# nvaccess/NVSpeechPlayer

Hardware: NVIDIA B200
Metric: audio-seconds synthesized/sec (batched streams) (higher is better)
Workload: dtype f32

## Files before the change

### nvspeechplayer_b200/csrc/host.cu

```cuda
#include <chrono>
#include <cstdio>
#include <mutex>
#include <vector>

#include "host.h"

using namespace klatt;

__global__ void init_states_kernel(StreamState *states, uint32_t n) {
	uint32_t i = blockIdx.x * blockDim.x + threadIdx.x;
	if (i >= n) return;
	states[i].fm.lastUserIndex = -1;
	states[i].fm.curIsNull = 1;
	states[i].fm.oldIsNull = 1;
}

namespace klatt {

thread_local std::string g_lastError;

int fail(const std::string &what) {
	g_lastError = what;
	if (envIs("NVSP_VERBOSE")) fprintf(stderr, "[nvspeechplayer_b200] %s\n", what.c_str());
	return -1;
}
void setLastError(const char *what) { fail(what ? what : "error"); }

bool cudaOk(cudaError_t e, const char *what) {
	if (e == cudaSuccess) return true;
	fail(std::string(what) + ": " + cudaGetErrorString(e));
	return false;
}

int pickDevice() {
	static const int chosen = envNum<int>("NVSP_DEVICE", -1);
	int dev = 0;
	if (chosen >= 0) {
		if (cudaSetDevice(chosen) != cudaSuccess) return -1;
		return chosen;
	}
	if (cudaGetDevice(&dev) != cudaSuccess) return -1;
	return dev;
}

int QueueBufs::upload(const void *hFrames, const uint32_t *hMin, const uint32_t *hFade, const int32_t *hUix, const uint8_t *hNull,
                      size_t n, cudaStream_t stream) {
	const size_t m = std::max<size_t>(n, 1);
	if ((hFrames && !frames.reserve(m * kNumParams * sizeof(double))) || (hMin && !minDur.reserve(m * 4)) ||
	    (hFade && !fadeDur.reserve(m * 4)) || (hUix && !userIndex.reserve(m * 4)) || (hNull && !isNull.reserve(m)))
		return -1;
	if (n == 0) return 0;
	if (hFrames) CU(cudaMemcpyAsync(frames.p, hFrames, n * kNumParams * sizeof(double), cudaMemcpyHostToDevice, stream));
	if (hMin) CU(cudaMemcpyAsync(minDur.p, hMin, n * 4, cudaMemcpyHostToDevice, stream));
	if (hFade) CU(cudaMemcpyAsync(fadeDur.p, hFade, n * 4, cudaMemcpyHostToDevice, stream));
	if (hUix) CU(cudaMemcpyAsync(userIndex.p, hUix, n * 4, cudaMemcpyHostToDevice, stream));
	if (hNull) CU(cudaMemcpyAsync(isNull.p, hNull, n, cudaMemcpyHostToDevice, stream));
	return 0;
}

cudaError_t initStates(StreamState *states, uint32_t n, cudaStream_t stream) {
	cudaError_t e = cudaMemsetAsync(states, 0, sizeof(StreamState) * (size_t)n, stream);
	if (e != cudaSuccess) return e;
	init_states_kernel<<<(n + 255) / 256, 256, 0, stream>>>(states, n);
	return cudaGetLastError();
}

bool RoundsCtx::init() {
	if (ok) return true;
	genTicks = std::max<uint32_t>(envNum<uint32_t>("NVSP_GEN_TICKS", 256) & ~63u, 64);
	holdTicks = std::max<uint32_t>(envNum<uint32_t>("NVSP_HOLD_TICKS", 512) & ~63u, 64);
	minStreams = envNum<uint32_t>("NVSP_ROUNDS_MIN_STREAMS", 2048);
	groups = std::min<uint32_t>(std::max<uint32_t>(envNum<uint32_t>("NVSP_GROUPS", 4), 1), kMaxGroups);
	persistent = !envIs("NVSP_SCHED", "rounds");
	blockSched = envIs("NVSP_SCHED", "block");
	blockHoldTicks = std::max<uint32_t>(envNum<uint32_t>("NVSP_BLOCK_HOLD_TICKS", 128) & ~63u, 64);
	blockMinStreams = envNum<uint32_t>("NVSP_BLOCK_MIN_STREAMS", 16384);
	schedGenTicks = std::max<uint32_t>(envNum<uint32_t>("NVSP_SCHED_GEN_TICKS", 384) & ~63u, 64);
	schedHoldTicks = std::max<uint32_t>(envNum<uint32_t>("NVSP_SCHED_HOLD_TICKS", 256) & ~63u, 64);
	schedHoldMax = std::max<uint32_t>(envNum<uint32_t>("NVSP_SCHED_HOLD_MAX", 4096) & ~63u, schedHoldTicks);
	schedFadeTicks = envNum<uint32_t>("NVSP_SCHED_FADE_TICKS", 0) & ~63u;
	schedFadeMax = std::min<uint32_t>(std::max<uint32_t>(envNum<uint32_t>("NVSP_SCHED_FADE_MAX", 512) & ~63u, schedFadeTicks), 4096);
	schedRoleSms = std::min<uint32_t>(envNum<uint32_t>("NVSP_SCHED_HOLD_SMS", 0), 255u) |
	               (std::min<uint32_t>(envNum<uint32_t>("NVSP_SCHED_FADE_SMS", 0), 255u) << 8);
	int dev = 0, sms = 0;
	cudaGetDevice(&dev);
	cudaDeviceGetAttribute(&sms, cudaDevAttrMultiProcessorCount, dev);
	const int perSm = klattF32SchedBlocksPerSm();
	schedBlocks = envNum<uint32_t>("NVSP_SCHED_BLOCKS", (uint32_t)(sms * std::max(perSm, 1)));
	blockBlocks = std::max<uint32_t>(envNum<uint32_t>("NVSP_BLOCK_BLOCKS", (uint32_t)sms), 1);
	if (envIs("NVSP_VERBOSE"))
		fprintf(stderr, "[nvspeechplayer_b200] scheduler: %d SMs x %d blocks, %u blocks, hold %u / general %u ticks\n", sms, perSm,
		        schedBlocks, schedHoldTicks, schedGenTicks);
	if (!cudaOk(cudaEventCreateWithFlags(&evStart, cudaEventDisableTiming), "cudaEventCreate")) return false;
	for (uint32_t g = 0; g < groups; ++g) {
		if (!cudaOk(cudaStreamCreateWithFlags(&lanes[2 * g], cudaStreamNonBlocking), "cudaStreamCreate")) return false;
		if (!cudaOk(cudaStreamCreateWithFlags(&lanes[2 * g + 1], cudaStreamNonBlocking), "cudaStreamCreate")) return false;
		if (!cudaOk(cudaEventCreateWithFlags(&evFork[g], cudaEventDisableTiming), "cudaEventCreate")) return false;
		if (!cudaOk(cudaEventCreateWithFlags(&evJoin[g], cudaEventDisableTiming), "cudaEventCreate")) return false;
	}
	ok = true;
	return true;
}

cudaError_t RoundsCtx::checkFault() {
	if (!hostFault.p) {
		if (hostFault.reserve(sizeof(uint32_t)) != cudaSuccess) return cudaErrorMemoryAllocation;
		*hostFault.as<uint32_t>() = 0;
	}
	return *hostFault.as<uint32_t>() ? cudaErrorLaunchTimeout : cudaSuccess;
}

RoundsCtx::~RoundsCtx() {
	if (evStart) cudaEventDestroy(evStart);
	for (uint32_t g = 0; g < kMaxGroups; ++g) {
		if (evFork[g]) cudaEventDestroy(evFork[g]);
		if (evJoin[g]) cudaEventDestroy(evJoin[g]);
		if (lanes[2 * g]) cudaStreamDestroy(lanes[2 * g]);
		if (lanes[2 * g + 1]) cudaStreamDestroy(lanes[2 * g + 1]);
	}
}

cudaError_t launchRender(int precision, const StreamDesc *descs, uint32_t n, int sampleRate, uint32_t sampleCount,
                         int16_t *out, size_t rowStride, uint32_t *written, StreamResult *results,
                         NoiseConfig noise, cudaStream_t stream, RoundsCtx *rc, bool planned, unsigned long long *launchCounter) {
	if (precision == kPrecisionF64) {
		if (launchCounter) ++*launchCounter;
		return launchKlattF64(descs, n, sampleRate, sampleCount, out, rowStride, written, results, noise, stream);
	}
	if (rc && planned && rc->init() && rc->blockSched && n >= rc->blockMinStreams && klattF32BlockCanTake(n, rc->blockBlocks)) {
		if (!rc->lite.reserve(klattF32BlockLiteBytes(n, rc->blockBlocks)) ||
		    !rc->scratchRow.reserve(sizeof(int16_t) * (size_t)std::max<uint32_t>(std::max(rc->schedHoldTicks, rc->holdTicks), rc->blockHoldTicks)))
			return cudaErrorMemoryAllocation;
		if (!rc->blockProf.p) {
			if (!rc->blockProf.reserve(256)) return cudaErrorMemoryAllocation;
			cudaMemsetAsync(rc->blockProf.p, 0, 256, stream);
		}
		if (cudaError_t e = rc->checkFault()) return e;
		return launchKlattF32Block(descs, n, sampleRate, sampleCount, rc->blockHoldTicks, out, rowStride, written, results, noise,
		                           rc->lite.p, rc->scratchRow.as<int16_t>(), rc->blockBlocks, rc->blockProf.p, rc->hostFault.as<uint32_t>(),
		                           stream, launchCounter);
	}
	if (rc && planned && rc->init() && rc->persistent && n >= rc->minStreams && sampleCount > rc->schedGenTicks) {
		uint32_t cap = 64;
		while (cap < 2 * n) cap <<= 1;
		if (cudaError_t e = rc->checkFault()) return e;
		if (!rc->ring.reserve(sizeof(uint32_t) * 3 * (size_t)cap) || !rc->ctl.reserve(2048) ||
		    !rc->scratchRow.reserve(sizeof(int16_t) * (size_t)std::max(std::max(std::max(rc->schedHoldTicks, rc->schedHoldMax), rc->holdTicks), rc->schedFadeMax)))
			return cudaErrorMemoryAllocation;
		if (klattF32SchedUsesLite() && !rc->lite.reserve(klattF32SchedLiteBytes(n, rc->schedBlocks))) return cudaErrorMemoryAllocation;
		return launchKlattF32Sched(descs, n, sampleRate, sampleCount, rc->schedHoldTicks, rc->schedGenTicks, out, rowStride, written,
		                           results, noise, rc->ring.as<uint32_t>(), cap, rc->ctl.p, rc->scratchRow.as<int16_t>(),
		                           rc->schedBlocks, rc->hostFault.as<uint32_t>(), rc->lite.p, rc->schedHoldMax, rc->schedFadeTicks,
		                           rc->schedFadeMax, rc->schedRoleSms, stream, launchCounter);
	}
	if (rc && planned && rc->init() && n >= rc->minStreams && sampleCount > rc->genTicks) {
		const uint32_t rounds = (sampleCount + rc->genTicks - 1) / rc->genTicks;
		if (!rc->listHold.reserve(sizeof(uint32_t) * (size_t)n) || !rc->listGen.reserve(sizeof(uint32_t) * (size_t)n) ||
		    !rc->counters.reserve(sizeof(uint32_t) * 2 * (size_t)rounds * rc->groups) ||
		    !rc->scratchRow.reserve(sizeof(int16_t) * (size_t)rc->holdTicks))
			return cudaErrorMemoryAllocation;
		return launchKlattF32Rounds(descs, n, sampleRate, sampleCount, rc->holdTicks, rc->genTicks, out, rowStride, written,
		                            results, noise, rc->listHold.as<uint32_t>(), rc->listGen.as<uint32_t>(),
		                            rc->counters.as<uint32_t>(), rc->scratchRow.as<int16_t>(), stream, rc->groups, rc->lanes, rc->evStart, rc->evFork,
		                            rc->evJoin, launchCounter);
	}
	if (launchCounter) ++*launchCounter;
	return launchKlattF32(descs, n, sampleRate, sampleCount, out, rowStride, written, results, noise, stream);
}

bool HostPipe::init() {
	if (ok) return true;
	if (!cudaOk(cudaStreamCreateWithFlags(&compute, cudaStreamNonBlocking), "cudaStreamCreate")) return false;
	if (!cudaOk(cudaStreamCreateWithFlags(&copy, cudaStreamNonBlocking), "cudaStreamCreate")) return false;
	for (int i = 0; i < 2; ++i) {
		if (!cudaOk(cudaEventCreateWithFlags(&kernelDone[i], cudaEventDisableTiming), "cudaEventCreate")) return false;
		if (!cudaOk(cudaEventCreateWithFlags(&copyDone[i], cudaEventDisableTiming), "cudaEventCreate")) return false;
	}
	ok = true;
	return true;
}

HostPipe::~HostPipe() {
	for (int i = 0; i < 2; ++i) {
		if (kernelDone[i]) cudaEventDestroy(kernelDone[i]);
		if (copyDone[i]) cudaEventDestroy(copyDone[i]);
	}
	if (compute) cudaStreamDestroy(compute);
	if (copy) cudaStreamDestroy(copy);
}

static size_t stagingBudgetBytes() {
	const size_t mb = envNum<size_t>("NVSP_STAGE_MB", 2048);
	return std::max<size_t>(mb, 1) << 20;
}

long long renderToHost(HostPipe &pipe, int precision, const StreamDesc *dDescs, uint32_t n, int sampleRate,
                       uint32_t sampleCount, int16_t *hostOut, uint32_t *perStream, StreamResult *lastResults,
                       NoiseConfig noise, unsigned long long *launchCounter, bool planned) {
	if (!pipe.init()) return -1;
	if (n == 0 || sampleCount == 0) return 0;
	size_t budget = stagingBudgetBytes();
	uint64_t maxTicks = std::max<uint64_t>(budget / ((size_t)n * sizeof(int16_t)), 8);
	uint32_t chunk = (uint32_t)std::min<uint64_t>(sampleCount, maxTicks);
	if (chunk < sampleCount) chunk = chunk >= 64 ? (chunk & ~63u) : (chunk & ~7u);
	size_t stride = ((size_t)chunk + 7) & ~(size_t)7;
	for (int i = 0; i < 2; ++i) {
		if (!pipe.stage[i].reserve(stride * n * sizeof(int16_t))) return -1;
		if (!pipe.res[i].reserve((size_t)n * sizeof(StreamResult))) return -1;
	}
	if (!cudaOk(pipe.hostRes.reserve(sizeof(StreamResult) * (size_t)n * 2), "cudaMallocHost")) return -1;
	StreamResult *hostRes = pipe.hostRes.as<StreamResult>();
	std::vector<uint32_t> total(n, 0);
	std::vector<uint32_t> chunkStart, chunkLen;
	{
		uint32_t len = chunk;
		if ((size_t)n * sampleCount * sizeof(int16_t) > ((size_t)256 << 20)) {
			uint64_t first = (((size_t)128 << 20) / ((size_t)n * sizeof(int16_t))) & ~(uint64_t)63;
			len = (uint32_t)std::min<uint64_t>(std::max<uint64_t>(first, 64), chunk);
		}
		for (uint32_t t = 0; t < sampleCount;) {
			uint32_t l = std::min(len, sampleCount - t);
			chunkStart.push_back(t); chunkLen.push_back(l);
			t += l;
			len = std::min<uint32_t>(len * 2, chunk >= 64 ? (chunk & ~63u) : chunk);
		}
	}
	const uint32_t numChunks = (uint32_t)chunkStart.size();
	const bool verbose = envIs("NVSP_VERBOSE");
	auto now = [] { return std::chrono::duration<double, std::milli>(std::chrono::steady_clock::now().time_since_epoch()).count(); };
	const double tStart = now();
	auto harvest = [&](uint32_t c) -> bool {
		int b = c & 1;
		if (!cudaOk(cudaEventSynchronize(pipe.copyDone[b]), "cudaEventSynchronize")) return false;
		const StreamResult *r = hostRes + (size_t)b * n;
		for (uint32_t s = 0; s < n; ++s) total[s] += r[s].written;
		if (lastResults && c + 1 == numChunks) memcpy(lastResults, r, sizeof(StreamResult) * (size_t)n);
		return true;
	};
	std::vector<cudaEvent_t> tev;
	if (verbose) {
		tev.resize(4 * (size_t)numChunks);
		for (auto &e : tev) cudaEventCreate(&e);
	}
	for (uint32_t c = 0; c < numChunks; ++c) {
		int b = c & 1;
		const uint32_t t0 = chunkStart[c], len = chunkLen[c];
		const double tA = now();
		if (c >= 2 && !harvest(c - 2)) return -1;
		const double tB = now();
		if (verbose) cudaEventRecord(tev[4 * c + 0], pipe.compute);
		CU(launchRender(precision, dDescs, n, sampleRate, len, pipe.stage[b].as<int16_t>(), stride, nullptr,
		                pipe.res[b].as<StreamResult>(), noise, pipe.compute, &pipe.rounds, planned, launchCounter));
		if (verbose) cudaEventRecord(tev[4 * c + 1], pipe.compute);
		CU(cudaEventRecord(pipe.kernelDone[b], pipe.compute));
		CU(cudaStreamWaitEvent(pipe.copy, pipe.kernelDone[b], 0));
		if (verbose) cudaEventRecord(tev[4 * c + 2], pipe.copy);
		CU(cudaMemcpy2DAsync(hostOut + t0, (size_t)sampleCount * sizeof(int16_t), pipe.stage[b].p,
		                     stride * sizeof(int16_t), (size_t)len * sizeof(int16_t), n, cudaMemcpyDeviceToHost, pipe.copy));
		CU(cudaMemcpyAsync(hostRes + (size_t)b * n, pipe.res[b].p, sizeof(StreamResult) * (size_t)n,
		                   cudaMemcpyDeviceToHost, pipe.copy));
		if (verbose) cudaEventRecord(tev[4 * c + 3], pipe.copy);
		CU(cudaEventRecord(pipe.copyDone[b], pipe.copy));
		if (verbose) fprintf(stderr, "[renderToHost] chunk %u/%u len %u: t=%.2f ms, waited %.2f ms for chunk-2, enqueue %.2f ms\n", c, numChunks, len,
		                     tA - tStart, tB - tA, now() - tB);
	}
	for (uint32_t c = (numChunks >= 2 ? numChunks - 2 : 0); c < numChunks; ++c)
		if (!harvest(c)) return -1;
	if (verbose) {
		fprintf(stderr, "[renderToHost] done at t=%.2f ms\n", now() - tStart);
		for (uint32_t c = 0; c < numChunks; ++c) {
			float k0, k1, c0, c1;
			cudaEventElapsedTime(&k0, tev[0], tev[4 * c + 0]); cudaEventElapsedTime(&k1, tev[0], tev[4 * c + 1]);
			cudaEventElapsedTime(&c0, tev[0], tev[4 * c + 2]); cudaEventElapsedTime(&c1, tev[0], tev[4 * c + 3]);
			fprintf(stderr, "[renderToHost]   chunk %u: kernel %.2f..%.2f ms, copy %.2f..%.2f ms\n", c, k0, k1, c0, c1);
		}
		for (auto &e : tev) cudaEventDestroy(e);
	}
	long long sum = 0;
	for (uint32_t s = 0; s < n; ++s) {
		sum += total[s];
		if (perStream) perStream[s] = total[s];
	}
	return sum;
}

}
```

### nvspeechplayer_b200/csrc/host.h

```cpp
#pragma once
#include <cuda_runtime.h>
#include <algorithm>
#include <cstdint>
#include <cstdlib>
#include <cstring>
#include <string>

#include "../../include/speechPlayer.h"
#include "klatt_common.h"
#include "launch.h"

namespace klatt {

static_assert(sizeof(speechPlayer_frame_t) == sizeof(double) * kNumParams, "a queued frame is kNumParams doubles");

extern thread_local std::string g_lastError;
int fail(const std::string &what);
void setLastError(const char *what);
bool cudaOk(cudaError_t e, const char *what);
#define CU(call) do { if (!cudaOk((call), #call)) return -1; } while (0)

template <class T = uint64_t> T envNum(const char *name, T dflt) {
	const char *e = getenv(name);
	return (e && *e) ? (T)strtoull(e, nullptr, 0) : dflt;
}
inline bool envIs(const char *name, const char *value = nullptr) {
	const char *e = getenv(name);
	return e && *e && (!value || strcmp(e, value) == 0);
}

int pickDevice();

struct DeviceGuard {
	int prev = -1;
	explicit DeviceGuard(int dev) {
		cudaGetDevice(&prev);
		if (prev != dev) cudaSetDevice(dev);
		else prev = -1;
	}
	~DeviceGuard() {
		if (prev >= 0) cudaSetDevice(prev);
	}
};

struct DevBuf {
	void *p = nullptr;
	size_t cap = 0;
	DevBuf() = default;
	DevBuf(const DevBuf &) = delete;
	DevBuf &operator=(const DevBuf &) = delete;
	DevBuf(DevBuf &&o) noexcept : p(o.p), cap(o.cap) { o.p = nullptr; o.cap = 0; }
	DevBuf &operator=(DevBuf &&o) noexcept { std::swap(p, o.p); std::swap(cap, o.cap); return *this; }
	~DevBuf() {
		if (p) cudaFree(p);
	}
	bool reserve(size_t bytes, const char *what = "cudaMalloc") {
		if (bytes <= cap) return true;
		size_t want = std::max(bytes, cap * 2);
		void *np = nullptr;
		if (!cudaOk(cudaMalloc(&np, want), what)) return false;
		if (p) cudaFree(p);
		p = np; cap = want;
		return true;
	}
	template <class T> T *as() const { return static_cast<T *>(p); }
};

struct PinnedBuf {
	void *p = nullptr;
	size_t cap = 0;
	PinnedBuf() = default;
	PinnedBuf(const PinnedBuf &) = delete;
	PinnedBuf &operator=(const PinnedBuf &) = delete;
	~PinnedBuf() {
		if (p) cudaFreeHost(p);
	}
	cudaError_t reserve(size_t bytes, unsigned flags = cudaHostAllocDefault) {
		if (bytes <= cap) return cudaSuccess;
		if (p) cudaFreeHost(p);
		p = nullptr; cap = 0;
		cudaError_t e = cudaHostAlloc(&p, bytes, flags);
		if (e == cudaSuccess) cap = bytes;
		else p = nullptr;
		return e;
	}
	template <class T> T *as() const { return static_cast<T *>(p); }
};

struct QueueBufs {
	DevBuf frames, minDur, fadeDur, userIndex, isNull;
	int upload(const void *hFrames, const uint32_t *hMin, const uint32_t *hFade, const int32_t *hUix, const uint8_t *hNull, size_t n,
	           cudaStream_t stream);
};

inline unsigned long long timelineTicks(const unsigned int *minDur, const unsigned int *fadeDur, size_t n) {
	unsigned long long t = 0;
	for (size_t i = 0; i < n; ++i) {
		unsigned long long m = minDur[i], f = fadeDur[i] > 1 ? fadeDur[i] : 1;
		t += std::max(m + 1, f + 2);
	}
	return t;
}

cudaError_t initStates(StreamState *states, uint32_t n, cudaStream_t stream);

struct RoundsCtx {
	static constexpr uint32_t kMaxGroups = 8;
	DevBuf listHold, listGen, counters, scratchRow;
	DevBuf ring, ctl;
	bool persistent = true;
	DevBuf lite, blockProf;
	bool blockSched = false;
	uint32_t blockHoldTicks = 128, blockMinStreams = 16384, blockBlocks = 0;
	PinnedBuf hostFault;
	uint32_t schedHoldTicks = 256, schedGenTicks = 384, schedHoldMax = 4096, schedFadeTicks = 0, schedFadeMax = 512, schedRoleSms = 0, schedBlocks = 0;
	cudaStream_t lanes[2 * kMaxGroups] = {};
	cudaEvent_t evStart = nullptr, evFork[kMaxGroups] = {}, evJoin[kMaxGroups] = {};
	uint32_t holdTicks = 512, genTicks = 256, minStreams = 2048, groups = 4;
	bool ok = false;
	bool init();
	cudaError_t checkFault();
	~RoundsCtx();
};

cudaError_t launchRender(int precision, const StreamDesc *descs, uint32_t n, int sampleRate, uint32_t sampleCount,
                         int16_t *out, size_t rowStride, uint32_t *written, StreamResult *results,
                         NoiseConfig noise, cudaStream_t stream, RoundsCtx *rc = nullptr, bool planned = false,
                         unsigned long long *launchCounter = nullptr);

struct HostPipe {
	cudaStream_t compute = nullptr, copy = nullptr;
	cudaEvent_t kernelDone[2] = {nullptr, nullptr}, copyDone[2] = {nullptr, nullptr};
	DevBuf stage[2], res[2];
	RoundsCtx rounds;
	PinnedBuf hostRes;
	bool ok = false;
	bool init();
	~HostPipe();
};

long long renderToHost(HostPipe &pipe, int precision, const StreamDesc *dDescs, uint32_t n, int sampleRate,
                       uint32_t sampleCount, int16_t *hostOut, uint32_t *perStream, StreamResult *lastResults,
                       NoiseConfig noise, unsigned long long *launchCounter, bool planned = false);

}
```

### nvspeechplayer_b200/csrc/klatt_f32_core.cuh

```cuda
#pragma once
#include <math.h>
#include <stdint.h>
#include <string.h>
#include <type_traits>
#include "klatt_common.h"
#include "philox.cuh"

#if defined(__GNUC__) || defined(__CUDACC__)
#define KLATT_UNLIKELY(x) __builtin_expect(!!(x), 0)
#else
#define KLATT_UNLIKELY(x) (x)
#endif

namespace klatt {

enum Direct : int {
	dVibratoPitchOffset = 0, dVoiceTurbulenceAmplitude, dGlottalOpenQuotient, dVoiceAmplitude,
	dAspirationAmplitude, dCaNP, dPa1, dPa2, dPa3, dPa4, dPa5, dPa6, dFricationAmplitude, dParallelBypass,
	dPreFormantGain, dOutputGain
};
static_assert(dOutputGain + 1 == kNumDirect, "direct slots");

KLATT_HD constexpr int directParam(int i) {
	return i == dVibratoPitchOffset ? kVibratoPitchOffset
	     : i == dVoiceTurbulenceAmplitude ? kVoiceTurbulenceAmplitude : i == dGlottalOpenQuotient ? kGlottalOpenQuotient
	     : i == dVoiceAmplitude ? kVoiceAmplitude : i == dAspirationAmplitude ? kAspirationAmplitude
	     : i == dCaNP ? kCaNP : i == dFricationAmplitude ? kFricationAmplitude
	     : (i >= dPa1 && i <= dPa6) ? (kPa1 + (i - dPa1))
	     : i == dParallelBypass ? kParallelBypass : i == dPreFormantGain ? kPreFormantGain : kOutputGain;
}

KLATT_HD void oneMinusExpD(double x, double th, double &re, double &im) {
	double em1 = expm1(x);
	double r = 1.0 + em1;
	double sh, ch;
	sincos(0.5 * th, &sh, &ch);
	re = -em1 + 2.0 * r * sh * sh;
	im = -r * (2.0 * sh * ch);
}
KLATT_HD void oneMinusExp(double x, double th, float &re, float &im) {
	double dre, dim;
	oneMinusExpD(x, th, dre, dim);
	re = (float)dre;
	im = (float)dim;
}
KLATT_HD void poleTerms(double f, double bw, double srInv, float &zre, float &zim) {
	const double PI = 3.14159265358979323846;
	oneMinusExp(-PI * bw * srInv , 2.0 * PI * f * srInv , zre, zim);
}

KLATT_HD int64_t vibratoIncrement(double speed, double srInv) {
	double t = speed * srInv;
	if (t != t) t = 0.0;
	if (!(t > -0.49 && t < 0.49)) t = fmod(t, 1.0);
	if (t >= 0.5) t -= 1.0;
	if (t < -0.5) t += 1.0;
	return (int64_t)(t * 18446744073709551616.0);
}

constexpr double kSinTurnsGain = 1.0 + 3.861e-8;
KLATT_HD double vibratoDepth(double vibratoPitchOffset) { return vibratoPitchOffset * (0.06 / kSinTurnsGain); }

KLATT_HD void planFade(const double *o, const double *n, uint32_t F, int sampleRate, FadePlanF32 &p) {
	const double srInv = 1.0 / (double)sampleRate;
	const double invF = 1.0 / (double)F;
	{
		double v0 = o[kVibratoSpeed], v1 = n[kVibratoSpeed];
		if (v1 != v1) v1 = v0;
		p.vibInc0 = vibratoIncrement(v0, srInv);
		p.vibIncFinal = vibratoIncrement(v0 + ((v1 - v0) * 1.0), srInv);
		p.vibIncStep = (p.vibIncFinal - p.vibInc0) / (int64_t)F;
		double d0 = o[kVibratoPitchOffset], d1 = n[kVibratoPitchOffset];
		if (d1 != d1) d1 = d0;
		p.depth0 = vibratoDepth(d0);
		p.depthStep = vibratoDepth((d1 - d0) * invF);
		p.depthFinal = vibratoDepth(d0 + ((d1 - d0) * 1.0));
	}
	for (int i = 0; i < kNumDirect; ++i) {
		double a = o[directParam(i)], b = n[directParam(i)];
		if (b != b) b = a;
		p.dir0[i] = (float)a;
		p.dirStep[i] = (float)((b - a) * invF);
		p.dirFinal[i] = (float)(a + ((b - a) * 1.0));
	}
	for (int r = 0; r < kNumResonators; ++r) {
		double f0 = o[resFreqParam(r)], f1 = n[resFreqParam(r)];
		double b0 = o[resBwParam(r)], b1 = n[resBwParam(r)];
		if (f1 != f1) f1 = f0;
		if (b1 != b1) b1 = b0;
		poleTerms(f0, b0, srInv, p.z0re[r], p.z0im[r]);
		poleTerms(f0 + ((f1 - f0) * 1.0), b0 + ((b1 - b0) * 1.0), srInv, p.zFre[r], p.zFim[r]);
		const double PI = 3.14159265358979323846;
		double xs = -PI * (b1 - b0) * invF * srInv;
		double dth = 2.0 * PI * (f1 - f0) * invF * srInv;
		double wr, wi;
		oneMinusExpD(xs, dth, wr, wi);
		p.wre[r] = (float)wr; p.wim[r] = (float)wi;
		static_assert(kCoarseTicks == 64, "six squarings");
#pragma unroll
		for (int k = 0; k < 6; ++k) {
			const double ar = 2.0 - wr, ai = -wi;
			const double nr = wr * ar - wi * ai, ni = wr * ai + wi * ar;
			wr = nr; wi = ni;
		}
		p.Wre[r] = (float)wr; p.Wim[r] = (float)wi;
		if (r == kResN0) {
			p.n0InvFade = !(f0 == 0 && f1 == 0);
			p.n0InvFinal = (f0 + ((f1 - f0) * 1.0)) != 0;
		}
	}
}

KLATT_HD void plannedFrames(const double *prevReal, bool prevIsNull, const double *cur, bool curIsNull, double *o, double *n) {
	for (int i = 0; i < kNumParams; ++i) o[i] = prevReal ? prevReal[i] : 0.0;
	if (prevIsNull) o[kPreFormantGain] = 0;
	if (curIsNull) {
		for (int i = 0; i < kNumParams; ++i) n[i] = o[i];
		n[kPreFormantGain] = 0;
	} else {
		for (int i = 0; i < kNumParams; ++i) n[i] = cur[i];
		if (prevIsNull) {
			for (int i = 0; i < kNumParams; ++i) o[i] = n[i];
			o[kPreFormantGain] = 0;
		}
	}
}

enum Role : int { kRoleBoth = 0, kRoleCascade = 1, kRoleParallel = 2, kRoleCascadeOsc = 3, kRoleParallelOnly = 4 };
constexpr int kGroupTicks = 8;
#ifndef KLATT_HOLD_UNROLL
#define KLATT_HOLD_UNROLL 1
#endif
constexpr int kHoldUnroll = KLATT_HOLD_UNROLL;

template <int ROLE> struct RoleTraits {
	static constexpr bool hasC = ROLE == kRoleBoth || ROLE == kRoleCascade || ROLE == kRoleCascadeOsc;
	static constexpr bool hasP = ROLE == kRoleBoth || ROLE == kRoleParallel || ROLE == kRoleParallelOnly;
	static constexpr bool hasO = ROLE == kRoleBoth || ROLE == kRoleParallel || ROLE == kRoleCascadeOsc;
	static constexpr int R0 = hasC ? 0 : kResParallel;
	static constexpr int R1 = hasP ? kNumResonators : kResParallel;
};
KLATT_HD constexpr bool directOfCascade(int i) {
	return i == dVoiceTurbulenceAmplitude || i == dGlottalOpenQuotient || i == dVoiceAmplitude ||
	       i == dAspirationAmplitude || i == dCaNP || i == dPreFormantGain || i == dOutputGain;
}
KLATT_HD constexpr bool directOfParallel(int i) {
	return i == dFricationAmplitude || (i >= dPa1 && i <= dPa6) || i == dParallelBypass || i == dPreFormantGain;
}
template <int ROLE> KLATT_HD constexpr bool roleUsesDirect(int i) {
	return (RoleTraits<ROLE>::hasC && directOfCascade(i)) || (RoleTraits<ROLE>::hasP && directOfParallel(i));
}

struct XchgSelf {
	uint32_t wA_;
	float par_, voice_;
	KLATT_HD void put(uint32_t, uint32_t wA, float par, float voice) { wA_ = wA; par_ = par; voice_ = voice; }
	KLATT_HD void get(uint32_t, uint32_t &wA, float &par, float &voice) const { wA = wA_; par = par_; voice = voice_; }
	KLATT_HD void sync() {}
};

struct F2 { float lo, hi; };
KLATT_HD F2 f2(float lo, float hi) { F2 r; r.lo = lo; r.hi = hi; return r; }
KLATT_HD F2 f2s(float x) { F2 r; r.lo = x; r.hi = x; return r; }
KLATT_HD F2 fma2(F2 a, F2 b, F2 c) {
	F2 r;
#ifdef __CUDA_ARCH__
	asm("{ .reg .b64 pa, pb, pc, pd; mov.b64 pa, {%2, %3}; mov.b64 pb, {%4, %5}; mov.b64 pc, {%6, %7}; "
	    "fma.rn.f32x2 pd, pa, pb, pc; mov.b64 {%0, %1}, pd; }"
	    : "=f"(r.lo), "=f"(r.hi) : "f"(a.lo), "f"(a.hi), "f"(b.lo), "f"(b.hi), "f"(c.lo), "f"(c.hi));
#else
	r.lo = fmaf(a.lo, b.lo, c.lo); r.hi = fmaf(a.hi, b.hi, c.hi);
#endif
	return r;
}
KLATT_HD F2 mul2(F2 a, F2 b) {
	F2 r;
#ifdef __CUDA_ARCH__
	asm("{ .reg .b64 pa, pb, pd; mov.b64 pa, {%2, %3}; mov.b64 pb, {%4, %5}; mul.rn.f32x2 pd, pa, pb; mov.b64 {%0, %1}, pd; }"
	    : "=f"(r.lo), "=f"(r.hi) : "f"(a.lo), "f"(a.hi), "f"(b.lo), "f"(b.hi));
#else
	r.lo = a.lo * b.lo; r.hi = a.hi * b.hi;
#endif
	return r;
}
KLATT_HD F2 add2(F2 a, F2 b) {
	F2 r;
#ifdef __CUDA_ARCH__
	asm("{ .reg .b64 pa, pb, pd; mov.b64 pa, {%2, %3}; mov.b64 pb, {%4, %5}; add.rn.f32x2 pd, pa, pb; mov.b64 {%0, %1}, pd; }"
	    : "=f"(r.lo), "=f"(r.hi) : "f"(a.lo), "f"(a.hi), "f"(b.lo), "f"(b.hi));
#else
	r.lo = a.lo + b.lo; r.hi = a.hi + b.hi;
#endif
	return r;
}
KLATT_HD F2 sub2(F2 a, F2 b) {
	F2 r;
#ifdef __CUDA_ARCH__
	asm("{ .reg .b64 pa, pb, pd; mov.b64 pa, {%2, %3}; mov.b64 pb, {%4, %5}; sub.rn.f32x2 pd, pa, pb; mov.b64 {%0, %1}, pd; }"
	    : "=f"(r.lo), "=f"(r.hi) : "f"(a.lo), "f"(a.hi), "f"(b.lo), "f"(b.hi));
#else
	r.lo = a.lo - b.lo; r.hi = a.hi - b.hi;
#endif
	return r;
}
KLATT_HD float &half(F2 *arr, int r) { return (r & 1) ? arr[r >> 1].hi : arr[r >> 1].lo; }
KLATT_HD const float &half(const F2 *arr, int r) { return (r & 1) ? arr[r >> 1].hi : arr[r >> 1].lo; }

constexpr int kNumPairs = kNumResonators / 2;
constexpr int kNumDirectPairs = kNumDirect / 2;
static_assert(kResCascade % 2 == 0 && kResParallel % 2 == 0, "role boundaries fall between pairs");
template <int ROLE> struct PairTraits {
	static constexpr int P0 = RoleTraits<ROLE>::R0 / 2, P1 = RoleTraits<ROLE>::R1 / 2;
};
template <int ROLE> KLATT_HD constexpr bool roleUsesDirectPair(int k) {
	return roleUsesDirect<ROLE>(2 * k) || roleUsesDirect<ROLE>(2 * k + 1);
}

struct DspState {
	F2 ny[kNumPairs];
	F2 d[kNumPairs];
	float aspLast, fricLast;
	uint64_t vibratoPos;
	int64_t vibInc;
	double pitchPos;
	double pitch, pitchInc;
	double depth;
};

struct CoefF32 {
	F2 a[kNumPairs], nrho[kNumPairs];
	float invA0;
	float vta, goq, va, aa, caNP, bypass;
	F2 pa[3];
	float halfGain, fricGain, og4000;
	bool n0Inv;
};

KLATT_HD float fastRcp(float x) {
#ifdef __CUDA_ARCH__
	float r;
	asm("rcp.approx.ftz.f32 %0, %1;" : "=f"(r) : "f"(x));
	return r;
#else
	return 1.0f / x;
#endif
}

constexpr float kDrawScale = 1.0f / 8388608.0f;

template <int ROLE>
KLATT_HD void buildCoef(CoefF32 &C, const F2 *u, const F2 *v, const F2 *dir, bool n0Inv) {
	using T = RoleTraits<ROLE>;
	using P = PairTraits<ROLE>;
#pragma unroll
	for (int k = P::P0; k < P::P1; ++k) {
		F2 a = fma2(u[k], u[k], mul2(v[k], v[k]));
		C.a[k] = a;
		C.nrho[k] = fma2(f2s(2.0f), u[k], a);
	}
	C.halfGain = half(dir, dPreFormantGain) * 0.5f;
	if (T::hasC) {
		C.invA0 = fastRcp(C.a[0].lo);
		C.vta = half(dir, dVoiceTurbulenceAmplitude); C.goq = half(dir, dGlottalOpenQuotient);
		C.va = half(dir, dVoiceAmplitude); C.aa = half(dir, dAspirationAmplitude); C.caNP = half(dir, dCaNP);
		C.og4000 = half(dir, dOutputGain) * 4000.0f;
		C.n0Inv = n0Inv;
	}
	if (T::hasP) {
		static_assert(dPa1 % 2 == 0, "the parallel amplitudes are whole pairs of the direct params");
#pragma unroll
		for (int k = 0; k < 3; ++k) C.pa[k] = dir[dPa1 / 2 + k];
		C.bypass = half(dir, dParallelBypass);
		C.fricGain = ((0.3f * kDrawScale) * half(dir, dFricationAmplitude)) * C.halfGain;
	}
}

template <int ROLE>
KLATT_HD void stepPoles(F2 *u, F2 *v, const F2 *wr, const F2 *wi) {
	using P = PairTraits<ROLE>;
#pragma unroll
	for (int k = P::P0; k < P::P1; ++k) {
		F2 zi = mul2(v[k], f2s(-1.0f));
		F2 tr = fma2(u[k], wr[k], wr[k]);
		tr = fma2(zi, wi[k], tr);
		F2 ti = fma2(u[k], wi[k], wi[k]);
		ti = fma2(v[k], wr[k], ti);
		u[k] = sub2(u[k], tr);
		v[k] = sub2(v[k], ti);
	}
}

KLATT_HD float sectionOut(float &ny, float &d, float a, float w, float x) {
	float dn = fmaf(a, x, w);
	d = dn;
	ny = ny - dn;
	return -ny;
}
KLATT_HD F2 sectionMemory(const DspState &S, const CoefF32 &C, int k) {
	F2 w = fma2(C.nrho[k], S.d[k], S.d[k]);
	return fma2(C.a[k], S.ny[k], w);
}

KLATT_HD float sinTurns(float t) {
	if (t > 0.25f) t = 0.5f - t;
	if (t < -0.25f) t = -0.5f - t;
	const float u = t * t;
	float q = fmaf(u, -14.3368558883667f, 41.999961853027344f);
	q = fmaf(u, q, -76.70366668701172f);
	q = fmaf(u, q, 81.60520935058594f);
	q = fmaf(u, q, -41.34170150756836f);
	return fmaf(t * u, q, t * 6.2831854820251465f);
}

KLATT_HD float bitsToFloat(uint32_t u) {
#ifdef __CUDA_ARCH__
	return __uint_as_float(u);
#else
	float f;
	memcpy(&f, &u, 4);
	return f;
#endif
}

KLATT_HD int64_t cyclesToFixed(double x) {
#ifdef __CUDA_ARCH__
	return __double2ll_rn(x * 18446744073709551616.0);
#else
	double y = x * 18446744073709551616.0;
	if (y != y) return (int64_t)0x8000000000000000ull;
	if (y >= 9223372036854775807.0) return 0x7fffffffffffffffll;
	if (y <= -9223372036854775808.0) return (int64_t)0x8000000000000000ull;
	return (int64_t)nearbyint(y);
#endif
}

KLATT_HD double fracRef(double x) {
#ifdef __CUDA_ARCH__
	if (fabs(x) < 2.0) {
		double t = x >= 1.0 ? 1.0 : 0.0;
		t = x <= -1.0 ? -1.0 : t;
		return x - t;
	}
	return x - (double)__double2int_rz(x);
#else
	double t = (x != x) ? 0.0 : (x >= 2147483647.0 ? 2147483647.0 : (x <= -2147483648.0 ? -2147483648.0 : (double)(int32_t)x));
	return x - t;
#endif
}

KLATT_HD double glideExact(double p, double inc, uint64_t n) {
	if (n == 0) return p;
	if (!(inc == inc) || !(p == p) || inc == 0.0) return p + inc;
	while (n > 0) {
		const double p1 = p + inc;
		if (--n == 0) return p1;
		const double p2 = p1 + inc;
		if (--n == 0) return p2;
		const double p3 = p2 + inc;
		--n;
		p = p3;
		if (n == 0) return p3;
		const double step = p3 - p2;
		if (step == 0.0) return p3;
		const double a1 = p1 < 0 ? -p1 : p1, a2 = p2 < 0 ? -p2 : p2, a3 = p3 < 0 ? -p3 : p3;
		if (!(a3 >= 1e-290 && a3 <= 1e290) || !(a2 >= 1e-290) || !(a1 >= 1e-290)) continue;
		int e1, e2, e3;
		(void)frexp(a1, &e1);
		(void)frexp(a2, &e2);
		const double f3 = frexp(a3, &e3);
		if (e1 != e3 || e2 != e3 || (p1 < 0) != (p3 < 0) || (p2 < 0) != (p3 < 0)) continue;
		const int64_t P = (int64_t)ldexp(f3, 53);
		const double sMag = ldexp(step, 53 - e3);
		const int64_t S = (p3 < 0) ? -(int64_t)sMag : (int64_t)sMag;
		if (S == 0) continue;
		const int64_t lo = (int64_t)1 << 52, hi = (int64_t)1 << 53;
		int64_t room = S > 0 ? (hi - P) / S : (P - lo) / (-S);
		room -= 1;
		if (room <= 0) continue;
		const uint64_t k = (uint64_t)room < n ? (uint64_t)room : n;
		const double mag = ldexp((double)(P + (int64_t)k * S), e3 - 53);
		p = (p3 < 0) ? -mag : mag;
		n -= k;
	}
	return p;
}

KLATT_HD float parallelSide(DspState &S, const CoefF32 &C, uint32_t wF) {
	float uF = bitsToFloat(0x4B000000u | (wF >> 9)) - 8388608.0f;
	S.fricLast = fmaf(0.75f, S.fricLast, uF);
	float pin = S.fricLast * C.fricGain;
	const F2 pin2 = f2s(pin);
	F2 nacc = f2s(0.0f);
#pragma unroll
	for (int k = 0; k < 3; ++k) {
		const int p = kResParallel / 2 + k;
		F2 dn = fma2(C.a[p], pin2, sectionMemory(S, C, p));
		S.d[p] = dn;
		S.ny[p] = sub2(S.ny[p], dn);
		nacc = fma2(add2(S.ny[p], pin2), C.pa[k], nacc);
	}
	float par = -(nacc.lo + nacc.hi);
	return fmaf(pin - par, C.bypass, par);
}

KLATT_HD double divideBySampleRate(double x, double srD, double srInv) {
	double q = x * srInv;
	double r = fma(-q, srD, x);
	return fma(r, srInv, q);
}

struct OscChain {
	float t, u, q;
	double m, quot, pos;
	KLATT_HD void seg1(DspState &S) {
		S.vibratoPos += (uint64_t)S.vibInc;
		t = (float)(int32_t)(uint32_t)(S.vibratoPos >> 32) * 2.3283064365386963e-10f;
		if (t > 0.25f) t = 0.5f - t;
		if (t < -0.25f) t = -0.5f - t;
		u = t * t;
	}
	KLATT_HD void seg2() {
		q = fmaf(u, -14.3368558883667f, 41.999961853027344f);
		q = fmaf(u, q, -76.70366668701172f);
		q = fmaf(u, q, 81.60520935058594f);
		q = fmaf(u, q, -41.34170150756836f);
		q = fmaf(t * u, q, t * 6.2831854820251465f);
	}
	KLATT_HD void seg3(DspState &S) {
		S.pitch += S.pitchInc;
		m = S.pitch * fma((double)q, S.depth, 1.0);
	}
	KLATT_HD void seg4(double srD, double srInv) { quot = divideBySampleRate(m, srD, srInv); }
	KLATT_HD void seg5(DspState &S) {
		pos = fracRef(quot + S.pitchPos);
		S.pitchPos = pos;
	}
	KLATT_HD float seg6() const { return (float)pos; }
};

KLATT_HD float oscillatorSide(DspState &S, const CoefF32 &C, double srD, double srInv) {
	OscChain o;
	o.seg1(S); o.seg2(); o.seg3(S); o.seg4(srD, srInv); o.seg5(S);
	return o.seg6();
}

KLATT_HD float stageSource(DspState &S, const CoefF32 &C, uint32_t wA, float voice) {
	float uA = bitsToFloat(0x4B000000u | (wA >> 9)) - 8388608.0f;
	S.aspLast = fmaf(0.75f, S.aspLast, uA);
	float asp = S.aspLast * (0.2f * kDrawScale);
	float turb = asp * C.vta;
	if (voice < C.goq) turb *= 0.01f;
	float v = (fmaf(voice, 2.0f, -1.0f) + turb) * C.va;
	float src = fmaf(asp, C.aa, v);
	return src * C.halfGain;
}
KLATT_HD float stageNasal(DspState &S, const CoefF32 &C, float ci) {
	float dx = ci - S.ny[0].lo;
	float dx1 = fmaf(C.nrho[0].lo, S.d[0].lo, S.d[0].lo);
	float n0 = C.n0Inv ? fmaf(dx - dx1, C.invA0, S.ny[0].lo)
	                   : fmaf(C.a[0].lo, dx, dx1 + S.ny[0].lo);
	S.d[0].lo = dx;
	S.ny[0].lo = ci;
	float wNP = fmaf(C.nrho[0].hi, S.d[0].hi, S.d[0].hi);
	wNP = fmaf(C.a[0].hi, S.ny[0].hi, wNP);
	float np = sectionOut(S.ny[0].hi, S.d[0].hi, C.a[0].hi, wNP, n0);
	return fmaf(np - ci, C.caNP, ci);
}
KLATT_HD float stageSection(DspState &S, const CoefF32 &C, int q, float w, float x) {
	const int r = kResCascade + q;
	return sectionOut(half(S.ny, r), half(S.d, r), half(C.a, r), w, x);
}
KLATT_HD int stageOut(const CoefF32 &C, float x, float par) {
	float s = (x + par) * C.og4000;
	s = fminf(s, 32000.0f);
	s = fmaxf(s, -32000.0f);
	return (int)s;
}

KLATT_HD int cascadeSide(DspState &S, const CoefF32 &C, uint32_t wA, float par, float voice) {
	float ci = stageSource(S, C, wA, voice);
	F2 w[3];
#pragma unroll
	for (int p = 0; p < 3; ++p) w[p] = sectionMemory(S, C, 1 + p);
	float x = stageNasal(S, C, ci);
#pragma unroll
	for (int q = 0; q < 6; ++q) x = stageSection(S, C, q, half(w, q), x);
	return stageOut(C, x, par);
}

struct NoiseSource {
	Philox4 blk;
	uint64_t blkIndex;
	KLATT_HD void init() { blk.w[0] = blk.w[1] = blk.w[2] = blk.w[3] = 0; blkIndex = ~0ull; }
	KLATT_HD void draw(const NoiseConfig &noise, const StreamDesc &desc, uint64_t streamId, uint64_t gen, uint32_t &wA, uint32_t &wF) {
		if (noise.mode == kNoisePhilox) {
			uint64_t b = gen >> 1;
			if (b != blkIndex) { blk = noiseBlock(noise.seed, streamId, b); blkIndex = b; }
			bool odd = (gen & 1ull) != 0;
			wA = odd ? blk.w[2] : blk.w[0];
			wF = odd ? blk.w[3] : blk.w[1];
		} else {
			uint64_t d0 = 2 * gen - desc.replayBase;
			wA = (d0 < desc.replayLen) ? ((uint32_t)desc.replay[d0] << 1) : 0u;
			wF = (d0 + 1 < desc.replayLen) ? ((uint32_t)desc.replay[d0 + 1] << 1) : 0u;
		}
	}
};

template <int ROLE, class GS>
KLATT_HD void loadDspState(DspState &S, const GS &gs) {
	using T = RoleTraits<ROLE>;
#pragma unroll
	for (int r = T::R0; r < T::R1; ++r) { half(S.ny, r) = (r == kResN0) ? gs.y[r] : -gs.y[r]; half(S.d, r) = gs.d[r]; }
	if (T::hasC) S.aspLast = gs.aspLast;
	if (T::hasP) S.fricLast = gs.fricLast;
	if (T::hasO) {
		S.vibratoPos = gs.vibratoPos; S.vibInc = gs.vibInc;
		S.pitchPos = gs.pitchPos; S.pitch = gs.pitch; S.pitchInc = gs.pitchInc; S.depth = gs.depth;
	}
}
template <int ROLE, class GS>
KLATT_HD void storeDspState(GS &gs, const DspState &S) {
	using T = RoleTraits<ROLE>;
#pragma unroll
	for (int r = T::R0; r < T::R1; ++r) { gs.y[r] = (r == kResN0) ? half(S.ny, r) : -half(S.ny, r); gs.d[r] = half(S.d, r); }
	if (T::hasC) gs.aspLast = S.aspLast;
	if (T::hasP) gs.fricLast = S.fricLast;
	if (T::hasO) {
		gs.vibratoPos = S.vibratoPos; gs.vibInc = S.vibInc;
		gs.pitchPos = S.pitchPos; gs.pitch = S.pitch; gs.pitchInc = S.pitchInc; gs.depth = S.depth;
	}
}

template <class FM, class GS>
KLATT_HD bool canHoldF32T(const FM &fm, const GS &gs, uint32_t ticks) {
	return !fm.hasNew && !fm.curIsNull && !fm.purgePending && gs.holdArmed && (uint64_t)fm.counter + ticks <= (uint64_t)fm.oldM;
}
KLATT_HD bool canHoldF32(const StreamState &st, uint32_t ticks) { return canHoldF32T(st.fm, st.gen.f32, ticks); }
template <class FM, class GS>
KLATT_HD bool canFadeF32T(const FM &fm, const GS &gs, uint32_t ticks) {
	return fm.hasNew && !fm.purgePending && fm.counter >= 1 && (uint64_t)fm.counter + ticks < (uint64_t)fm.newF &&
	       (gs.samplesGenerated & (uint64_t)(kCoarseTicks - 1)) == 0;
}

template <int ROLE, class Out, class Xchg, class FM, class GS>
KLATT_HD void renderHoldF32T(FM &fm, GS &gs, const StreamDesc &desc, int sampleRate, uint32_t ticks, Out &out, const NoiseConfig &noise,
                             Xchg &xc) {
	using T = RoleTraits<ROLE>;
	const double srD = (double)sampleRate, srInv = 1.0 / (double)sampleRate;
	DspState S;
	loadDspState<ROLE>(S, gs);
	CoefF32 C;
	{
		F2 u[kNumPairs], v[kNumPairs], dir[kNumDirectPairs];
#pragma unroll
		for (int r = T::R0; r < T::R1; ++r) { half(u, r) = -gs.zre[r]; half(v, r) = -gs.zim[r]; }
#pragma unroll
		for (int i = 0; i < kNumDirect; ++i)
			if (roleUsesDirectPair<ROLE>(i / 2)) half(dir, i) = roleUsesDirect<ROLE>(i) ? gs.dir[i] : 0.0f;
		buildCoef<ROLE>(C, u, v, dir, gs.n0Inv != 0);
	}
	uint64_t gen = gs.samplesGenerated;
	const uint64_t streamId = desc.streamId;
	NoiseSource ns;
	ns.init();
	const bool evenPhilox = noise.mode == kNoisePhilox && (gen & 1ull) == 0;
	for (uint32_t t = 0; t < ticks; t += kGroupTicks) {
		if (T::hasC && !T::hasP) xc.sync();
		if (!T::hasP || evenPhilox) {
#pragma unroll(kHoldUnroll)
			for (int k = 0; k < kGroupTicks; k += 2) {
				Philox4 blk;
				if (T::hasP) blk = noiseBlock(noise.seed, streamId, (gen + k) >> 1);
#pragma unroll
				for (int h = 0; h < 2; ++h) {
					uint32_t wA = 0;
					float par = 0.0f, voice = 0.0f;
					if (T::hasP) {
						wA = blk.w[2 * h];
						par = parallelSide(S, C, blk.w[2 * h + 1]);
						if (T::hasO && !T::hasC) voice = oscillatorSide(S, C, srD, srInv);
						if (!T::hasC) xc.put(t + k + h, wA, par, voice);
					}
					if (T::hasC) {
						if (!T::hasP) xc.get(t + k + h, wA, par, voice);
						if (T::hasO) voice = oscillatorSide(S, C, srD, srInv);
						out.push(cascadeSide(S, C, wA, par, voice));
					}
				}
			}
		} else {
			for (int k = 0; k < kGroupTicks; ++k) {
				uint32_t wA, wF;
				ns.draw(noise, desc, streamId, gen + k, wA, wF);
				float par = parallelSide(S, C, wF), voice = 0.0f;
				if (T::hasO) voice = oscillatorSide(S, C, srD, srInv);
				if (!T::hasC) xc.put(t + k, wA, par, voice);
				if (T::hasC) out.push(cascadeSide(S, C, wA, par, voice));
			}
		}
		gen += kGroupTicks;
		if (T::hasP && !T::hasC) xc.sync();
	}
	storeDspState<ROLE>(gs, S);
	if (T::hasC) {
		gs.samplesGenerated = gen;
		fm.counter += ticks;
		gs.callPos += ticks;
	}
}
template <int ROLE, class Out, class Xchg>
KLATT_HD void renderHoldF32(const StreamDesc &desc, int sampleRate, uint32_t ticks, Out &out, const NoiseConfig &noise, Xchg &xc) {
	renderHoldF32T<ROLE>(desc.state->fm, desc.state->gen.f32, desc, sampleRate, ticks, out, noise, xc);
}

template <int ROLE, class Out, class Xchg, class FM, class GS>
KLATT_HD uint32_t renderGeneralF32T(FM &fm, GS &gs, const StreamDesc &desc, int sampleRate, uint32_t myTicks, uint32_t loopTicks, Out &out,
                                    const NoiseConfig &noise, Xchg &xc, int32_t *lastUserIndexOut, uint32_t *qHeadOut) {
	using T = RoleTraits<ROLE>;
	constexpr bool kInline = ROLE == kRoleBoth && std::is_same<FM, FrameMgrState>::value;
	const double srD = (double)sampleRate, srInv = 1.0 / (double)sampleRate;
	const bool planned = desc.plans != nullptr;

	uint32_t counter = fm.counter, qHead = fm.qHead;
	uint32_t oldM = fm.oldM, newM = fm.newM, newF = fm.newF;
	int32_t lastUserIndex = fm.lastUserIndex;
	bool hasNew = fm.hasNew, curIsNull = fm.curIsNull, oldIsNull = fm.oldIsNull, newIsNull = fm.newIsNull;
	uint32_t nextEvent = gs.nextEvent;
	bool holdArmed = gs.holdArmed != 0;
	bool n0Inv = gs.n0Inv != 0;

	DspState S;
	loadDspState<ROLE>(S, gs);
	using P = PairTraits<ROLE>;
	F2 u[kNumPairs], v[kNumPairs], wr[kNumPairs], wi[kNumPairs];
	F2 dir0[kNumDirectPairs], dstep[kNumDirectPairs];
	float kf = 0.0f, kfStep = 0.0f;
	int64_t vibIncStep = 0;
	double depthStep = 0.0;
#pragma unroll
	for (int r = T::R0; r < T::R1; ++r) { half(u, r) = -gs.zre[r]; half(v, r) = -gs.zim[r]; half(wr, r) = 0.0f; half(wi, r) = 0.0f; }
#pragma unroll
	for (int i = 0; i < kNumDirect; ++i)
		if (roleUsesDirectPair<ROLE>(i / 2)) { half(dir0, i) = roleUsesDirect<ROLE>(i) ? gs.dir[i] : 0.0f; half(dstep, i) = 0.0f; }
	uint64_t gen = gs.samplesGenerated;
	const uint64_t streamId = desc.streamId;

	if constexpr (kInline) {
		if (fm.purgePending) {
			fm.purgePending = 0;
			counter = oldM;
			if (hasNew) {
				oldIsNull = newIsNull;
				for (int i = 0; i < kNumParams; ++i) fm.oldFrame[i] = fm.curFrame[i];
				hasNew = false;
			}
			S.pitchInc = 0.0;
			holdArmed = false;
			nextEvent = oldM + 1;
		}
	}
	const FadePlanF32 *plan = nullptr;
	if (hasNew) {
		if constexpr (kInline) plan = planned ? desc.plans + (qHead - 1 - desc.qBase) : &gs.plan;
		else plan = desc.plans + (qHead - 1 - desc.qBase);
		if (counter >= 1 && counter < newF) {
#pragma unroll
			for (int r = T::R0; r < T::R1; ++r) { half(wr, r) = plan->wre[r]; half(wi, r) = plan->wim[r]; }
#pragma unroll
			for (int i = 0; i < kNumDirect; ++i)
				if (roleUsesDirect<ROLE>(i)) { half(dir0, i) = plan->dir0[i]; half(dstep, i) = plan->dirStep[i]; }
			kf = (float)counter;
			kfStep = 1.0f;
			vibIncStep = plan->vibIncStep;
			depthStep = plan->depthStep;
		}
	}
	uint32_t coarseAt = hasNew ? gs.coarseAt : 0x80000000u;

	NoiseSource ns;
	ns.init();

	uint32_t produced = 0;
	bool active = myTicks > 0;
	for (uint32_t tg = 0; tg < loopTicks; tg += kGroupTicks) {
	if (T::hasC && !T::hasP) xc.sync();
	for (uint32_t t = tg; t < tg + kGroupTicks && t < loopTicks; ++t) {
		if (active) {
			counter++;
			if (KLATT_UNLIKELY(counter >= nextEvent)) {
				if (hasNew) {
					if (counter > newF) {
						if constexpr (kInline) {
							if (!planned)
								for (int i = 0; i < kNumParams; ++i) fm.oldFrame[i] = fm.newFrame[i];
						}
						oldM = newM; oldIsNull = newIsNull;
						if (T::hasO) fm.oldInc = fm.newInc;
						hasNew = false;
						S.pitchInc = 0.0;
						nextEvent = counter + 1;
					} else if (counter == 1 && newF > 1) {
#pragma unroll
						for (int r = T::R0; r < T::R1; ++r) {
							half(u, r) = -plan->z0re[r]; half(v, r) = -plan->z0im[r]; half(wr, r) = plan->wre[r]; half(wi, r) = plan->wim[r];
						}
#pragma unroll
						for (int i = 0; i < kNumDirect; ++i)
							if (roleUsesDirect<ROLE>(i)) { half(dir0, i) = plan->dir0[i]; half(dstep, i) = plan->dirStep[i]; }
						kf = 0.0f; kfStep = 1.0f;
						if (T::hasO) {
							S.vibInc = plan->vibInc0; vibIncStep = plan->vibIncStep;
							S.depth = plan->depth0; depthStep = plan->depthStep;
							const double pitchOld = gs.pitchOld, pitchNew = gs.pitchNew;
							S.pitch = pitchOld;
							S.pitchInc = (pitchNew != pitchNew) ? 0.0 : (pitchNew - pitchOld) / (double)newF;
						}
						if (T::hasC) n0Inv = plan->n0InvFade != 0;
						coarseAt = 0x80000000u;
						nextEvent = newF;
					} else {
#pragma unroll
						for (int r = T::R0; r < T::R1; ++r) {
							half(u, r) = -plan->zFre[r]; half(v, r) = -plan->zFim[r]; half(wr, r) = 0.0f; half(wi, r) = 0.0f;
						}
#pragma unroll
						for (int i = 0; i < kNumDirect; ++i)
							if (roleUsesDirect<ROLE>(i)) { half(dir0, i) = plan->dirFinal[i]; half(dstep, i) = 0.0f; }
						kf = 0.0f; kfStep = 0.0f;
						if (T::hasC) n0Inv = plan->n0InvFinal != 0;
						if (T::hasO) {
							const double pitchOld = gs.pitchOld, pitchNew = gs.pitchNew;
							S.pitch = (pitchNew != pitchNew) ? pitchOld : pitchOld + ((pitchNew - pitchOld) * 1.0);
							S.pitchInc = 0.0;
							S.vibInc = plan->vibIncFinal; vibIncStep = 0;
							S.depth = plan->depthFinal; depthStep = 0.0;
						}
						nextEvent = newF + 1;
					}
				} else if (counter > oldM) {
					uint32_t rel = qHead - desc.qBase;
					if (rel < desc.qCount) {
						curIsNull = false;
						newM = desc.minDur[rel];
						uint32_t fd = desc.fadeDur[rel];
						newF = fd > 1u ? fd : 1u;
						newIsNull = desc.isNull ? (desc.isNull[rel] != 0) : false;
						int32_t ux = desc.userIndex ? desc.userIndex[rel] : -1;
						qHead++;
						hasNew = true;
						double pitchOld = S.pitch, pitchNew, newInc;
						if constexpr (kInline) {
							if (!planned) {
								fm.oldFrame[kVoicePitch] = S.pitch;
								for (int i = 0; i < kNumParams; ++i) fm.curFrame[i] = fm.oldFrame[i];
							}
						}
						if (newIsNull) {
							if constexpr (kInline) {
								if (!planned) {
									for (int i = 0; i < kNumParams; ++i) fm.newFrame[i] = fm.oldFrame[i];
									fm.newFrame[kPreFormantGain] = 0;
								}
							}
							pitchNew = S.pitch;
							newInc = 0;
						} else {
							const double *fr = desc.frames + (size_t)rel * kNumParams;
							pitchNew = fr[kVoicePitch];
							newInc = (fr[kEndVoicePitch] - fr[kVoicePitch]) / (double)newM;
							if constexpr (kInline) {
								if (!planned)
									for (int i = 0; i < kNumParams; ++i) fm.newFrame[i] = fr[i];
							}
							if (oldIsNull) {
								pitchOld = pitchNew;
								if constexpr (kInline) {
									if (!planned) {
										for (int i = 0; i < kNumParams; ++i) fm.oldFrame[i] = fm.newFrame[i];
										fm.oldFrame[kPreFormantGain] = 0;
									}
								}
							}
						}
						if (ux != -1) lastUserIndex = ux;
						counter = 0;
						pitchNew += (newInc * (double)newF);
						if (T::hasO) { gs.pitchOld = pitchOld; gs.pitchNew = pitchNew; fm.newInc = newInc; }
						if (planned) {
							plan = desc.plans + rel;
						} else {
							if constexpr (kInline) {
								fm.newFrame[kVoicePitch] = pitchNew;
								fm.oldFrame[kVoicePitch] = pitchOld;
								planFade(fm.oldFrame, fm.newFrame, newF, sampleRate, gs.plan);
								plan = &gs.plan;
							}
						}
						S.pitchInc = 0.0;
						holdArmed = false;
						nextEvent = 1;
					} else {
						curIsNull = true;
					}
				} else {
					if (T::hasO) S.pitchInc = fm.oldInc;
					holdArmed = true;
					nextEvent = oldM + 1;
				}
				if (curIsNull) active = false;
			}
		}
		if (active) {
			uint32_t wA = 0, wF = 0;
			if (T::hasP) ns.draw(noise, desc, streamId, gen, wA, wF);
			const bool oscHere = T::hasO && !T::hasC;
			OscChain osc;
			kf += kfStep;
			if (T::hasO) { S.vibInc += vibIncStep; S.depth += depthStep; }
			if (KLATT_UNLIKELY((gen & (uint64_t)(kCoarseTicks - 1)) == 0 && kfStep != 0.0f)) {
				if (counter - coarseAt == (uint32_t)kCoarseTicks) {
#pragma unroll
					for (int r = T::R0; r < T::R1; ++r) {
						float zr = gs.zc[r], zi = gs.zc[kNumResonators + r], Wr = plan->Wre[r], Wi = plan->Wim[r];
						float tr = fmaf(-zr, Wr, Wr);
						tr = fmaf(zi, Wi, tr);
						float ti = fmaf(-zr, Wi, Wi);
						ti = fmaf(-zi, Wr, ti);
						half(u, r) = -(zr + tr);
						half(v, r) = -(zi + ti);
					}
				} else {
					stepPoles<ROLE>(u, v, wr, wi);
				}
#pragma unroll
				for (int r = T::R0; r < T::R1; ++r) { gs.zc[r] = -half(u, r); gs.zc[kNumResonators + r] = -half(v, r); }
				coarseAt = counter;
			} else {
				stepPoles<ROLE>(u, v, wr, wi);
			}
			if (oscHere) { osc.seg1(S); osc.seg2(); }
			CoefF32 C;
			{
				F2 dir[kNumDirectPairs];
				const F2 kf2 = f2s(kf);
#pragma unroll
				for (int k = 0; k < kNumDirectPairs; ++k)
					if (roleUsesDirectPair<ROLE>(k)) dir[k] = fma2(kf2, dstep[k], dir0[k]);
				if (oscHere) osc.seg3(S);
				buildCoef<ROLE>(C, u, v, dir, n0Inv);
			}
			if (oscHere) osc.seg4(srD, srInv);
			float par = 0.0f, voice = 0.0f;
			if (T::hasP) {
				if (oscHere) osc.seg5(S);
				par = parallelSide(S, C, wF);
				if (oscHere) voice = osc.seg6();
				if (!T::hasC) xc.put(t, wA, par, voice);
			}
			gen++;
			if (T::hasC) {
				if (!T::hasP) xc.get(t, wA, par, voice);
				if (T::hasO) voice = oscillatorSide(S, C, srD, srInv);
				out.push(cascadeSide(S, C, wA, par, voice));
			}
			produced++;
			if (produced == myTicks) active = false;
		}
	}
	if (T::hasP && !T::hasC) xc.sync();
	}

	if constexpr (kInline) {
		if (!planned) {
			if (hasNew) {
				if (counter >= 1) {
					double ratio = (double)counter / (double)newF;
					for (int i = 0; i < kNumParams; ++i) {
						double o = fm.oldFrame[i], n = fm.newFrame[i];
						fm.curFrame[i] = (n != n) ? o : o + ((n - o) * ratio);
					}
				}
			} else {
				for (int i = 0; i < kNumParams; ++i) fm.curFrame[i] = fm.oldFrame[i];
				fm.oldFrame[kVoicePitch] = S.pitch;
			}
			fm.curFrame[kVoicePitch] = S.pitch;
		}
	}
	storeDspState<ROLE>(gs, S);
#pragma unroll
	for (int r = T::R0; r < T::R1; ++r) { gs.zre[r] = -half(u, r); gs.zim[r] = -half(v, r); }
#pragma unroll
	for (int i = 0; i < kNumDirect; ++i)
		if (roleUsesDirect<ROLE>(i) && (T::hasC || i != dPreFormantGain)) gs.dir[i] = fmaf(kf, half(dstep, i), half(dir0, i));
	if (T::hasC) {
		fm.counter = counter; fm.qHead = qHead; fm.oldM = oldM; fm.newM = newM; fm.newF = newF;
		fm.lastUserIndex = lastUserIndex;
		fm.hasNew = hasNew; fm.curIsNull = curIsNull; fm.oldIsNull = oldIsNull; fm.newIsNull = newIsNull;
		gs.n0Inv = n0Inv ? 1u : 0u;
		gs.holdArmed = holdArmed ? 1u : 0u;
		gs.nextEvent = nextEvent;
		gs.samplesGenerated = gen;
		gs.coarseAt = coarseAt;
		gs.callPos += produced;
		if (produced < myTicks) gs.callDrained = 1;
	}
	*lastUserIndexOut = lastUserIndex;
	*qHeadOut = qHead;
	return produced;
}
template <int ROLE, class Out, class Xchg>
KLATT_HD uint32_t renderGeneralF32(const StreamDesc &desc, int sampleRate, uint32_t myTicks, uint32_t loopTicks, Out &out,
                                   const NoiseConfig &noise, Xchg &xc, int32_t *lastUserIndexOut, uint32_t *qHeadOut) {
	return renderGeneralF32T<ROLE>(desc.state->fm, desc.state->gen.f32, desc, sampleRate, myTicks, loopTicks, out, noise, xc,
	                               lastUserIndexOut, qHeadOut);
}

template <int ROLE, class Out, class Xchg, class FM, class GS>
KLATT_HD void renderFadeF32T(FM &fm, GS &gs, const StreamDesc &desc, int sampleRate, uint32_t ticks, Out &out, const NoiseConfig &noise,
                             Xchg &xc) {
	using T = RoleTraits<ROLE>;
	const double srD = (double)sampleRate, srInv = 1.0 / (double)sampleRate;
	const uint32_t rel = fm.qHead - 1u - desc.qBase;
	const FadePlanF32 *plan = desc.plans + (rel < desc.qCount ? rel : 0u);
	uint32_t counter = fm.counter;
	DspState S;
	loadDspState<ROLE>(S, gs);
	F2 u[kNumPairs], v[kNumPairs], wr[kNumPairs], wi[kNumPairs];
	F2 dir0[kNumDirectPairs], dstep[kNumDirectPairs];
#pragma unroll
	for (int r = T::R0; r < T::R1; ++r) { half(u, r) = -gs.zre[r]; half(v, r) = -gs.zim[r]; half(wr, r) = plan->wre[r]; half(wi, r) = plan->wim[r]; }
#pragma unroll
	for (int i = 0; i < kNumDirect; ++i)
		if (roleUsesDirectPair<ROLE>(i / 2)) {
			half(dir0, i) = roleUsesDirect<ROLE>(i) ? plan->dir0[i] : 0.0f;
			half(dstep, i) = roleUsesDirect<ROLE>(i) ? plan->dirStep[i] : 0.0f;
		}
	float kf = (float)counter;
	const int64_t vibIncStep = plan->vibIncStep;
	const double depthStep = plan->depthStep;
	const bool n0Inv = gs.n0Inv != 0;
	uint64_t gen = gs.samplesGenerated;
	const uint64_t streamId = desc.streamId;
	uint32_t coarseAt = gs.coarseAt;
#pragma unroll 1
	for (uint32_t c0 = 0; c0 < ticks; c0 += (uint32_t)kCoarseTicks) {
		const uint32_t cellTicks = ticks - c0 < (uint32_t)kCoarseTicks ? ticks - c0 : (uint32_t)kCoarseTicks;
		{
			if (counter + 1u - coarseAt == (uint32_t)kCoarseTicks) {
#pragma unroll
				for (int r = T::R0; r < T::R1; ++r) {
					float zr = gs.zc[r], zi = gs.zc[kNumResonators + r], Wr = plan->Wre[r], Wi = plan->Wim[r];
					float tr = fmaf(-zr, Wr, Wr);
					tr = fmaf(zi, Wi, tr);
					float ti = fmaf(-zr, Wi, Wi);
					ti = fmaf(-zi, Wr, ti);
					half(u, r) = -(zr + tr);
					half(v, r) = -(zi + ti);
				}
			} else {
				stepPoles<ROLE>(u, v, wr, wi);
			}
#pragma unroll
			for (int r = T::R0; r < T::R1; ++r) { gs.zc[r] = -half(u, r); gs.zc[kNumResonators + r] = -half(v, r); }
		}
		coarseAt = counter + 1u;
		for (uint32_t t = 0; t < cellTicks; t += kGroupTicks) {
			if (T::hasC && !T::hasP) xc.sync();
#pragma unroll 1
			for (int k = 0; k < kGroupTicks; k += 2) {
				Philox4 blk;
				if (T::hasP) blk = noiseBlock(noise.seed, streamId, (gen + k) >> 1);
#pragma unroll
				for (int h = 0; h < 2; ++h) {
					const bool oscHere = T::hasO && !T::hasC;
					OscChain osc;
					counter++;
					kf += 1.0f;
					if (T::hasO) { S.vibInc += vibIncStep; S.depth += depthStep; }
					if (t + k + h != 0) stepPoles<ROLE>(u, v, wr, wi);
					if (oscHere) { osc.seg1(S); osc.seg2(); }
					CoefF32 C;
					{
						F2 dir[kNumDirectPairs];
						const F2 kf2 = f2s(kf);
#pragma unroll
						for (int q = 0; q < kNumDirectPairs; ++q)
							if (roleUsesDirectPair<ROLE>(q)) dir[q] = fma2(kf2, dstep[q], dir0[q]);
						if (oscHere) osc.seg3(S);
						buildCoef<ROLE>(C, u, v, dir, n0Inv);
					}
					if (oscHere) osc.seg4(srD, srInv);
					uint32_t wA = 0;
					float par = 0.0f, voice = 0.0f;
					if (T::hasP) {
						wA = blk.w[2 * h];
						if (oscHere) osc.seg5(S);
						par = parallelSide(S, C, blk.w[2 * h + 1]);
						if (oscHere) voice = osc.seg6();
						if (!T::hasC) xc.put(t + k + h, wA, par, voice);
					}
					if (T::hasC) {
						if (!T::hasP) xc.get(t + k + h, wA, par, voice);
						if (T::hasO) voice = oscillatorSide(S, C, srD, srInv);
						out.push(cascadeSide(S, C, wA, par, voice));
					}
				}
			}
			gen += kGroupTicks;
			if (T::hasP && !T::hasC) xc.sync();
		}
	}
	storeDspState<ROLE>(gs, S);
#pragma unroll
	for (int r = T::R0; r < T::R1; ++r) { gs.zre[r] = -half(u, r); gs.zim[r] = -half(v, r); }
#pragma unroll
	for (int i = 0; i < kNumDirect; ++i)
		if (roleUsesDirect<ROLE>(i) && (T::hasC || i != dPreFormantGain)) gs.dir[i] = fmaf(kf, half(dstep, i), half(dir0, i));
	if (T::hasC) {
		fm.counter = counter;
		gs.samplesGenerated = gen;
		gs.coarseAt = coarseAt;
		gs.callPos += ticks;
	}
}

}
```

### nvspeechplayer_b200/csrc/klatt_f32_sched.cu

```cuda
#include <cuda_runtime.h>
#include <stdio.h>
#include <stdlib.h>
#include <stddef.h>
#include <string.h>
#include "klatt_common.h"
#include "klatt_f32_core.cuh"
#include "out_writer.cuh"
#include "klatt_f32_pair.cuh"
#include "launch.h"

#ifndef KLATT_SCHED_LITE
#define KLATT_SCHED_LITE 1
#endif

namespace klatt {

#ifdef KLATT_SCHED_PROFILE
#define PROF_LAP(acc) { long long t1 = clock64(); acc += t1 - t0; t0 = t1; }
#else
#define PROF_LAP(acc)
#endif

constexpr uint32_t kRingEmpty = 0xffffffffu, kRingAbandoned = 0xfffffffeu;
constexpr uint32_t kClassHold = 0, kClassGen = 1, kClassFade = 2, kClassExit = 3, kNumRings = 3;

struct SchedCtl {
	uint32_t head0, padA[31];
	uint32_t head1, padB[31];
	uint32_t tail0, padC[31];
	uint32_t tail1, padD[31];
	uint32_t remaining, padE[31];
	uint32_t fault, padF[31];
	uint32_t head2, padG[31];
	uint32_t tail2, padH[31];
	__device__ __forceinline__ uint32_t *head(uint32_t c) { return c == 0 ? &head0 : c == 1 ? &head1 : &head2; }
	__device__ __forceinline__ uint32_t *tail(uint32_t c) { return c == 0 ? &tail0 : c == 1 ? &tail1 : &tail2; }
};

constexpr unsigned long long kWatchdogNs = 20ull * 1000 * 1000 * 1000;

namespace {

__device__ __forceinline__ unsigned long long globalTimerNs() {
	unsigned long long t;
	asm volatile("mov.u64 %0, %%globaltimer;" : "=l"(t));
	return t;
}

__device__ __forceinline__ uint32_t ldVolatile(const uint32_t *p) { return *reinterpret_cast<const volatile uint32_t *>(p); }
__device__ __forceinline__ void stVolatile(uint32_t *p, uint32_t v) { *reinterpret_cast<volatile uint32_t *>(p) = v; }

template <class FM, class GS>
__device__ __forceinline__ uint32_t classifyNextT(const FM &fm, const GS &gs, uint32_t sampleCount, uint32_t holdTicks, uint32_t fadeTicks) {
	const uint32_t pos = gs.callPos;
	if (pos >= sampleCount || gs.callDrained != 0) return kClassExit;
	if (sampleCount - pos >= holdTicks && canHoldF32T(fm, gs, holdTicks)) return kClassHold;
	if (fadeTicks != 0u && sampleCount - pos >= fadeTicks && canFadeF32T(fm, gs, fadeTicks)) return kClassFade;
	return kClassGen;
}
__device__ __forceinline__ uint32_t classifyNext(const StreamState *st, uint32_t sampleCount, uint32_t holdTicks) {
	return classifyNextT(st->fm, st->gen.f32, sampleCount, holdTicks, 0u);
}
constexpr uint32_t kRecPieces = sizeof(StreamStateLite) / 16, kStageStride = sizeof(StreamStateLite) + 8, kStageBytes = 32 * kStageStride;
constexpr uint32_t kHoldPiecesOut = (uint32_t)(offsetof(StreamStateLite, f32) + offsetof(GenStateF32Lite, zre)) / 16;
static_assert((offsetof(StreamStateLite, f32) + offsetof(GenStateF32Lite, zre)) % 16 == 0, "the hold chunk's write-back ends on a 16-byte piece");

template <bool SEED>
__device__ __forceinline__ void schedPush(SchedCtl *ctl, uint32_t *ring, uint32_t ringCap, uint32_t cls, uint32_t s, bool valid) {
	const unsigned lane = threadIdx.x & 31u, below = (1u << lane) - 1u;
	const unsigned mH = __ballot_sync(0xffffffffu, valid && cls == kClassHold);
	const unsigned mG = __ballot_sync(0xffffffffu, valid && cls == kClassGen);
	const unsigned mF = __ballot_sync(0xffffffffu, valid && cls == kClassFade);
	const unsigned mX = __ballot_sync(0xffffffffu, valid && cls == kClassExit);
	uint32_t baseH = 0, baseG = 0, baseF = 0;
	if (lane == 0) {
		if (mH) baseH = atomicAdd(ctl->tail(kClassHold), (uint32_t)__popc(mH));
		if (mG) baseG = atomicAdd(ctl->tail(kClassGen), (uint32_t)__popc(mG));
		if (mF) baseF = atomicAdd(ctl->tail(kClassFade), (uint32_t)__popc(mF));
	}
	baseH = __shfl_sync(0xffffffffu, baseH, 0);
	baseG = __shfl_sync(0xffffffffu, baseG, 0);
	baseF = __shfl_sync(0xffffffffu, baseF, 0);
	const uint32_t mask = ringCap - 1u;
	if (valid && cls != kClassExit) {
		uint32_t *r = ring + cls * ringCap;
		uint32_t idx = cls == kClassHold ? baseH + __popc(mH & below) : cls == kClassGen ? baseG + __popc(mG & below) : baseF + __popc(mF & below);
		if (SEED) {
			stVolatile(r + (idx & mask), s);
		} else {
			while (atomicCAS(r + (idx & mask), kRingEmpty, s) != kRingEmpty) {
				stVolatile(r + (idx & mask), kRingEmpty);
				idx = atomicAdd(ctl->tail(cls), 1u);
			}
		}
	}
	if (SEED) {
		if (lane == 0 && (mH | mG | mF)) atomicAdd(&ctl->remaining, (uint32_t)__popc(mH | mG | mF));
	} else {
		if (lane == 0 && mX) atomicSub(&ctl->remaining, (uint32_t)__popc(mX));
	}
}

__device__ __forceinline__ uint32_t schedClaim(SchedCtl *ctl, uint32_t *ring, uint32_t ringCap, uint32_t &s, uint32_t primary) {
	const unsigned lane = threadIdx.x & 31u;
	const uint32_t mask = ringCap - 1u;
	for (;;) {
		uint32_t cls = kClassExit, base = 0;
		if (lane == 0) {
			uint32_t backoff = 128;
			unsigned long long idleSince = 0;
			for (;;) {
				int32_t b0 = (int32_t)(ldVolatile(&ctl->tail0) - ldVolatile(&ctl->head0));
				int32_t b1 = (int32_t)(ldVolatile(&ctl->tail1) - ldVolatile(&ctl->head1));
				int32_t b2 = (int32_t)(ldVolatile(&ctl->tail2) - ldVolatile(&ctl->head2));
				if (b0 > 0 || b1 > 0 || b2 > 0) {
					uint32_t pick = kClassGen;
					int32_t best = -1;
					bool bestFull = false;
					auto consider = [&](uint32_t c, int32_t backlog, int32_t score) {
						if (backlog <= 0) return;
						const bool full = backlog >= 32;
						if (best < 0 || (full && !bestFull) || (full == bestFull && score > best)) { pick = c; best = score; bestFull = full; }
					};
					consider(kClassGen, b1, 2 * b1);
					consider(kClassFade, b2, 2 * b2);
					consider(kClassHold, b0, b0);
					if (primary < kNumRings) {
						const int32_t bp = primary == kClassHold ? b0 : primary == kClassGen ? b1 : b2;
						if (bp >= 32 || (bp > 0 && !bestFull)) pick = primary;
					}
					cls = pick;
					base = atomicAdd(ctl->head(cls), 32u);
					break;
				}
				if (ldVolatile(&ctl->remaining) == 0u) break;
				__nanosleep(backoff);
				if (backoff < 4096u) {
					backoff *= 2u;
				} else {
					const unsigned long long now = globalTimerNs();
					if (idleSince == 0) idleSince = now;
					else if (now - idleSince > kWatchdogNs) {
						stVolatile(&ctl->fault, 1u);
						stVolatile(&ctl->remaining, 0u);
					}
				}
			}
		}
		cls = __shfl_sync(0xffffffffu, cls, 0);
		base = __shfl_sync(0xffffffffu, base, 0);
		if (cls == kClassExit) return kClassExit;
		uint32_t *slot = ring + cls * ringCap + ((base + lane) & mask);
		s = kRingEmpty;
		bool abandoned = false;
		for (uint32_t spins = 0;; ++spins) {
			if (s == kRingEmpty && !abandoned) {
				const uint32_t v = ldVolatile(slot);
				if (v < kRingAbandoned) { s = v; stVolatile(slot, kRingEmpty); }
			}
			const unsigned got = __ballot_sync(0xffffffffu, s != kRingEmpty);
			const unsigned open = __ballot_sync(0xffffffffu, s == kRingEmpty && !abandoned);
			if (open == 0u) {
				if (got) return cls;
				break;
			}
			uint32_t quit = 0;
			if (lane == 0) {
				if (got) quit = spins >= 64u;
				else if ((spins & 15u) == 15u)
				{
					quit = ldVolatile(&ctl->remaining) == 0u;
					for (uint32_t c = 0; c < kNumRings; ++c)
						if (c != cls && (int32_t)(ldVolatile(ctl->tail(c)) - ldVolatile(ctl->head(c))) >= 32) quit = 1u;
				}
			}
			quit = __shfl_sync(0xffffffffu, quit, 0);
			if (quit) {
				if (s == kRingEmpty && !abandoned) {
					const uint32_t v = atomicCAS(slot, kRingEmpty, kRingAbandoned);
					if (v < kRingAbandoned) { s = v; stVolatile(slot, kRingEmpty); }
					else abandoned = true;
				}
			} else {
				__nanosleep(160);
			}
		}
	}
}

}

__global__ void __launch_bounds__(256)
klatt_sched_seed_kernel(const StreamDesc *__restrict__ descs, const StreamStateLite *__restrict__ lite, uint32_t numStreams,
                        uint32_t sampleCount, uint32_t holdTicks, uint32_t fadeTicks, SchedCtl *ctl, uint32_t *ring, uint32_t ringCap) {
	const uint32_t s = blockIdx.x * blockDim.x + threadIdx.x;
	const bool valid = s < numStreams;
	uint32_t cls = kClassExit;
	if (valid) {
		if (lite) {
			cls = classifyNextT(lite[s].fm, lite[s].f32, sampleCount, holdTicks, fadeTicks);
		} else {
			StreamState *st = descs[s].state;
			st->gen.f32.callPos = 0;
			st->gen.f32.callDrained = 0;
			cls = classifyNext(st, sampleCount, holdTicks);
		}
	}
	schedPush<true>(ctl, ring, ringCap, cls, s, valid);
}

#ifndef KLATT_SCHED_MINB
#define KLATT_SCHED_MINB 4
#endif
__global__ void __launch_bounds__(kPairBlock, KLATT_SCHED_MINB)
klatt_f32_sched_kernel(const StreamDesc *__restrict__ descs, StreamStateLite *__restrict__ lite, uint32_t numStreams, int sampleRate,
                       uint32_t sampleCount, uint32_t holdTicks, uint32_t genTicks, int16_t *__restrict__ out, size_t rowStride,
                       int16_t *__restrict__ scratchRow, NoiseConfig noise, SchedCtl *ctl, uint32_t *ring, uint32_t ringCap,
                       uint32_t roleSms, uint32_t holdMax, uint32_t fadeTicks, uint32_t fadeMax) {
	extern __shared__ uint4 schedSmem[];
	uint4 (*xbuf)[2 * kGroupTicks * 32] = reinterpret_cast<uint4 (*)[2 * kGroupTicks * 32]>(schedSmem);
	__shared__ uint32_t work[2][34];
	const uint32_t warp = threadIdx.x >> 5, lane = threadIdx.x & 31u, pair = warp & 1u;
	const bool cascade = cascadeRole(warp);
	XchgSmem xc{(uint32_t)__cvta_generic_to_shared(&xbuf[pair][lane]), 1u + pair};
#if KLATT_SCHED_LITE
	unsigned char *stage = reinterpret_cast<unsigned char *>(schedSmem + 2 * 2 * kGroupTicks * 32) + pair * kStageBytes;
	StreamStateLite *st = reinterpret_cast<StreamStateLite *>(stage + lane * kStageStride);
	StreamStateLite *dummy = lite + numStreams + (size_t)blockIdx.x * 2 + pair;
	const uint32_t tw = (warp >> 1) * 32u + lane;
#endif
#ifdef KLATT_SCHED_PROFILE
	long long tClaim = 0, tHold = 0, tGen = 0, tFade = 0, tPush = 0, nHold = 0, nGen = 0, nLanes = 0;
	long long t0 = clock64();
#endif
	uint32_t primary = kClassExit;
	if (roleSms) {
		uint32_t smid, nsm;
		asm("mov.u32 %0, %%smid;" : "=r"(smid));
		asm("mov.u32 %0, %%nsmid;" : "=r"(nsm));
		const uint32_t nH = roleSms & 0xffu, nF = roleSms >> 8;
		if ((smid + 1) * nH / nsm != smid * nH / nsm) {
			primary = kClassHold;
		} else {
			const uint32_t j = smid - smid * nH / nsm, rest = nsm > nH ? nsm - nH : 1u;
			primary = ((j + 1) * nF / rest != j * nF / rest) ? kClassFade : kClassGen;
		}
	}
	for (;;) {
		if (cascade) {
			uint32_t s = kRingEmpty;
			const uint32_t cls = schedClaim(ctl, ring, ringCap, s, primary);
			if (s == kRingEmpty) s = numStreams;
			__threadfence();
			work[pair][lane] = s;
			if (lane == 0) work[pair][32] = cls;
		}
		xc.sync();
		const uint32_t s = work[pair][lane], cls = work[pair][32];
		PROF_LAP(tClaim)
		if (cls == kClassExit) break;
		const bool valid = s < numStreams;
		const StreamDesc &desc = descs[s];
#if KLATT_SCHED_LITE
#pragma unroll 1
		for (uint32_t idx = tw; idx < 32u * kRecPieces; idx += 64u) {
			const uint32_t r = idx / kRecPieces, p = idx - r * kRecPieces;
			const uint32_t sr = work[pair][r];
			const StreamStateLite *src = sr < numStreams ? lite + sr : dummy;
			const uint4 v = __ldcg(reinterpret_cast<const uint4 *>(src) + p);
			uint2 *dst = reinterpret_cast<uint2 *>(stage + r * kStageStride + p * 16u);
			dst[0] = make_uint2(v.x, v.y);
			dst[1] = make_uint2(v.z, v.w);
		}
		xc.sync();
		FrameMgrLite &fm = st->fm;
		GenStateF32Lite &gs = st->f32;
#else
		FrameMgrState &fm = desc.state->fm;
		GenStateF32 &gs = desc.state->gen.f32;
#endif
		if (cls == kClassHold) {
			uint32_t ticks = holdTicks;
#if KLATT_SCHED_LITE
			if (holdMax > holdTicks) {
				uint32_t can = 0xffffffffu;
				if (valid) {
					const uint32_t left = sampleCount - gs.callPos, quiet = fm.oldM - fm.counter;
					can = left < quiet ? left : quiet;
				}
				can = __reduce_min_sync(0xffffffffu, can);
				if (can > holdMax) can = holdMax;
				can &= ~63u;
				if (can > ticks) ticks = can;
			}
#endif
			if (cascade) {
				int16_t *row = valid ? out + (size_t)s * rowStride + gs.callPos : scratchRow;
				OutWriter ow;
				ow.init(row, ((reinterpret_cast<uintptr_t>(row) & 15u) == 0));
				renderHoldF32T<kRoleCascadeOsc>(fm, gs, desc, sampleRate, ticks, ow, noise, xc);
			} else {
				NullOut no;
				renderHoldF32T<kRoleParallelOnly>(fm, gs, desc, sampleRate, ticks, no, noise, xc);
			}
		} else if (cls == kClassFade) {
			uint32_t ticks = fadeTicks;
			if (fadeMax > fadeTicks) {
				uint32_t can = 0xffffffffu;
				if (valid) {
					const uint32_t left = sampleCount - gs.callPos, inside = fm.newF - 1u - fm.counter;
					can = left < inside ? left : inside;
				}
				can = __reduce_min_sync(0xffffffffu, can);
				if (can > fadeMax) can = fadeMax;
				can &= ~63u;
				if (can > ticks) ticks = can;
			}
			if (cascade) {
				int16_t *row = valid ? out + (size_t)s * rowStride + gs.callPos : scratchRow;
				OutWriter ow;
				ow.init(row, ((reinterpret_cast<uintptr_t>(row) & 15u) == 0));
				renderFadeF32T<kRoleCascade>(fm, gs, desc, sampleRate, ticks, ow, noise, xc);
			} else {
				NullOut no;
				renderFadeF32T<kRoleParallel>(fm, gs, desc, sampleRate, ticks, no, noise, xc);
			}
		} else {
			const uint32_t pos = gs.callPos;
			uint32_t ticks = 0;
			if (valid) {
				ticks = sampleCount - pos;
				if (ticks > genTicks) ticks = genTicks;
				if (fadeTicks != 0u) {
					const uint64_t end = gs.samplesGenerated + ticks, grid = end & ~(uint64_t)(kCoarseTicks - 1);
					if (grid > gs.samplesGenerated && pos + ticks < sampleCount) ticks = (uint32_t)(grid - gs.samplesGenerated);
				}
			}
			int32_t lastUserIndex;
			uint32_t qHead;
			if (cascade) {
				int16_t *row = out + (size_t)(valid ? s : 0) * rowStride;
				OutWriter ow;
				ow.init(row + pos, ((reinterpret_cast<uintptr_t>(row + pos) & 15u) == 0));
				const uint32_t produced = renderGeneralF32T<kRoleCascade>(fm, gs, desc, sampleRate, ticks, genTicks, ow, noise, xc, &lastUserIndex, &qHead);
				ow.flush();
				if (produced < ticks) zeroRow(row, pos + produced, sampleCount);
			} else {
				NullOut no;
				renderGeneralF32T<kRoleParallel>(fm, gs, desc, sampleRate, ticks, genTicks, no, noise, xc, &lastUserIndex, &qHead);
			}
		}
#if KLATT_SCHED_LITE
		xc.sync();
		const uint32_t next = (cascade && valid) ? classifyNextT(fm, gs, sampleCount, holdTicks, fadeTicks) : kClassExit;
		const uint32_t piecesOut = cls == kClassHold ? kHoldPiecesOut : kRecPieces;
#pragma unroll 1
		for (uint32_t idx = tw; idx < 32u * piecesOut; idx += 64u) {
			const uint32_t r = idx / piecesOut, p = idx - r * piecesOut;
			const uint32_t sr = work[pair][r];
			if (sr < numStreams) {
				const uint2 *src = reinterpret_cast<const uint2 *>(stage + r * kStageStride + p * 16u);
				const uint2 a = src[0], b = src[1];
				__stcg(reinterpret_cast<uint4 *>(lite + sr) + p, make_uint4(a.x, a.y, b.x, b.y));
			}
		}
#endif
		__threadfence();
		xc.sync();
#ifdef KLATT_SCHED_PROFILE
		if (cls == kClassHold) { PROF_LAP(tHold) nHold++; } else if (cls == kClassFade) { PROF_LAP(tFade) nGen++; } else { PROF_LAP(tGen) nGen++; }
		nLanes += __popc(__ballot_sync(0xffffffffu, valid));
#endif
		if (cascade) {
#if !KLATT_SCHED_LITE
			const uint32_t next = valid ? classifyNext(desc.state, sampleCount, holdTicks) : kClassExit;
#endif
			schedPush<false>(ctl, ring, ringCap, next, s, valid);
		}
		PROF_LAP(tPush)
	}
#ifdef KLATT_SCHED_PROFILE
	if (lane == 0) {
		unsigned long long *p = reinterpret_cast<unsigned long long *>(ctl) + 128 + (cascade ? 0 : 8);
		atomicAdd(p + 0, (unsigned long long)tClaim); atomicAdd(p + 1, (unsigned long long)tHold);
		atomicAdd(p + 2, (unsigned long long)tGen); atomicAdd(p + 3, (unsigned long long)tPush);
		atomicAdd(p + 4, (unsigned long long)nHold); atomicAdd(p + 5, (unsigned long long)nGen);
		atomicAdd(p + 6, (unsigned long long)nLanes); atomicAdd(p + 7, (unsigned long long)tFade);
	}
#endif
}

static size_t schedSmemBytes() {
	return sizeof(uint4) * 2 * 2 * kGroupTicks * 32 + (KLATT_SCHED_LITE ? 2 * (size_t)kStageBytes : 0);
}
bool klattF32SchedUsesLite() { return KLATT_SCHED_LITE != 0; }
size_t klattF32SchedLiteBytes(uint32_t numStreams, uint32_t numBlocks) {
	return sizeof(StreamStateLite) * ((size_t)numStreams + 2 * (size_t)numBlocks);
}

cudaError_t launchKlattF32Sched(const StreamDesc *descs, uint32_t numStreams, int sampleRate, uint32_t sampleCount,
                                uint32_t holdTicks, uint32_t genTicks, int16_t *out, size_t rowStride, uint32_t *samplesWritten,
                                StreamResult *results, NoiseConfig noise, uint32_t *ring, uint32_t ringCap, void *ctlMem,
                                int16_t *scratchRow, uint32_t numBlocks, uint32_t *hostFault, void *liteMem, uint32_t holdMax,
                                uint32_t fadeTicks, uint32_t fadeMax, uint32_t roleSms, cudaStream_t stream, unsigned long long *launchCounter) {
	if (numStreams == 0 || sampleCount == 0) return cudaSuccess;
	SchedCtl *ctl = static_cast<SchedCtl *>(ctlMem);
	StreamStateLite *lite = KLATT_SCHED_LITE ? static_cast<StreamStateLite *>(liteMem) : nullptr;
	static bool attrSet = false;
	if (!attrSet) {
		cudaError_t ea = cudaFuncSetAttribute(klatt_f32_sched_kernel, cudaFuncAttributeMaxDynamicSharedMemorySize, (int)schedSmemBytes());
		if (ea != cudaSuccess) return ea;
		attrSet = true;
	}
	if (!lite) fadeTicks = 0;
	cudaError_t e = cudaMemsetAsync(ring, 0xff, sizeof(uint32_t) * kNumRings * (size_t)ringCap, stream);
	if (e != cudaSuccess) return e;
	if ((e = cudaMemsetAsync(ctl, 0, 2048, stream)) != cudaSuccess) return e;
	const uint32_t batches = (numStreams + 31) / 32;
	const uint32_t blocksWanted = (batches + 1) / 2, grid = blocksWanted < numBlocks ? blocksWanted : numBlocks;
	if (lite && (e = launchKlattLiteImport(descs, numStreams, 2 * grid, lite, stream)) != cudaSuccess) return e;
	klatt_sched_seed_kernel<<<(numStreams + 255) / 256, 256, 0, stream>>>(descs, lite, numStreams, sampleCount, holdTicks, fadeTicks, ctl, ring, ringCap);
	static const bool l2Persist = getenv("NVSP_L2_PERSIST") && atoi(getenv("NVSP_L2_PERSIST")) != 0;
	bool windowSet = false;
	if (lite && l2Persist) {
		int dev = 0, maxPersist = 0, maxWindow = 0;
		cudaGetDevice(&dev);
		cudaDeviceGetAttribute(&maxPersist, cudaDevAttrMaxPersistingL2CacheSize, dev);
		cudaDeviceGetAttribute(&maxWindow, cudaDevAttrMaxAccessPolicyWindowSize, dev);
		const size_t bytes = klattF32SchedLiteBytes(numStreams, grid);
		if (maxPersist > 0 && maxWindow > 0) {
			static size_t limitSet = 0;
			const size_t wantLimit = bytes < (size_t)maxPersist ? bytes : (size_t)maxPersist;
			if (wantLimit > limitSet && cudaDeviceSetLimit(cudaLimitPersistingL2CacheSize, wantLimit) == cudaSuccess) limitSet = wantLimit;
			cudaStreamAttrValue attr;
			memset(&attr, 0, sizeof attr);
			attr.accessPolicyWindow.base_ptr = lite;
			attr.accessPolicyWindow.num_bytes = bytes < (size_t)maxWindow ? bytes : (size_t)maxWindow;
			attr.accessPolicyWindow.hitRatio = limitSet >= bytes ? 1.0f : (float)((double)limitSet / (double)bytes);
			attr.accessPolicyWindow.hitProp = cudaAccessPropertyPersisting;
			attr.accessPolicyWindow.missProp = cudaAccessPropertyStreaming;
			windowSet = cudaStreamSetAttribute(stream, cudaStreamAttributeAccessPolicyWindow, &attr) == cudaSuccess;
			if (!windowSet) cudaGetLastError();
		}
	}
	klatt_f32_sched_kernel<<<grid, kPairBlock, schedSmemBytes(), stream>>>(descs, lite, numStreams, sampleRate, sampleCount, holdTicks, genTicks,
	                                                                        out, rowStride, scratchRow, noise, ctl, ring, ringCap, roleSms, holdMax, fadeTicks, fadeMax);
	if (windowSet) {
		cudaStreamAttrValue attr;
		memset(&attr, 0, sizeof attr);
		attr.accessPolicyWindow.num_bytes = 0;
		cudaStreamSetAttribute(stream, cudaStreamAttributeAccessPolicyWindow, &attr);
	}
	if (hostFault && (e = cudaMemcpyAsync(hostFault, &ctl->fault, sizeof(uint32_t), cudaMemcpyDeviceToHost, stream)) != cudaSuccess) return e;
	if (lite) {
		if ((e = launchKlattLiteExport(descs, numStreams, lite, samplesWritten, results, stream)) != cudaSuccess) return e;
		if (launchCounter) *launchCounter += 4;
	} else {
		if ((e = launchKlattFinalize(descs, numStreams, samplesWritten, results, stream)) != cudaSuccess) return e;
		if (launchCounter) *launchCounter += 3;
	}
#ifdef KLATT_SCHED_PROFILE
	{
		unsigned long long h[16];
		cudaStreamSynchronize(stream);
		cudaMemcpy(h, reinterpret_cast<unsigned long long *>(ctl) + 128, sizeof(h), cudaMemcpyDeviceToHost);
		for (int k = 0; k < 2; ++k)
			fprintf(stderr, "[sched profile] %s warps: claim %.1f  hold %.1f  gen %.1f  fade %.1f  push %.1f Mcycles; batches hold %llu gen+fade %llu; lanes/batch %.2f\n",
			        k ? "parallel" : "cascade ", h[8 * k] / 1e6, h[8 * k + 1] / 1e6, h[8 * k + 2] / 1e6, h[8 * k + 7] / 1e6, h[8 * k + 3] / 1e6, h[8 * k + 4], h[8 * k + 5],
			        (double)h[8 * k + 6] / (double)(h[8 * k + 4] + h[8 * k + 5]));
	}
#endif
	return cudaGetLastError();
}

int klattF32SchedBlocksPerSm() {
	int n = 0;
	cudaFuncSetAttribute(klatt_f32_sched_kernel, cudaFuncAttributeMaxDynamicSharedMemorySize, (int)schedSmemBytes());
	if (cudaOccupancyMaxActiveBlocksPerMultiprocessor(&n, klatt_f32_sched_kernel, kPairBlock, schedSmemBytes()) != cudaSuccess) n = 0;
	return n;
}

}
```

### nvspeechplayer_b200/csrc/launch.h

```cpp
#pragma once
#include <cuda_runtime.h>
#include <stddef.h>
#include <stdint.h>
#include "klatt_common.h"

namespace klatt {

struct PullState;
struct PullCtx;
struct PullSeg;
struct PullBatchItem;
struct PhaseChunk;

cudaError_t launchKlattF64(const StreamDesc *descs, uint32_t numStreams, int sampleRate, uint32_t sampleCount,
                           int16_t *out, size_t rowStride, uint32_t *samplesWritten, StreamResult *results,
                           NoiseConfig noise, cudaStream_t stream);

cudaError_t launchKlattF32(const StreamDesc *descs, uint32_t numStreams, int sampleRate, uint32_t sampleCount,
                           int16_t *out, size_t rowStride, uint32_t *samplesWritten, StreamResult *results,
                           NoiseConfig noise, cudaStream_t stream);
cudaError_t launchKlattF32Rounds(const StreamDesc *descs, uint32_t numStreams, int sampleRate, uint32_t sampleCount,
                                 uint32_t holdTicks, uint32_t genTicks, int16_t *out, size_t rowStride,
                                 uint32_t *samplesWritten, StreamResult *results, NoiseConfig noise, uint32_t *listHold,
                                 uint32_t *listGen, uint32_t *counters, int16_t *scratchRow, cudaStream_t stream, uint32_t numGroups,
                                 cudaStream_t *lanes, cudaEvent_t evStart, cudaEvent_t *evFork, cudaEvent_t *evJoin,
                                 unsigned long long *launchCounter);
cudaError_t launchKlattFinalize(const StreamDesc *descs, uint32_t numStreams, uint32_t *samplesWritten, StreamResult *results,
                                cudaStream_t stream);
cudaError_t launchKlattPlan(const int64_t *offsets, uint32_t numStreams, uint64_t totalRequests, const double *frames,
                            const uint32_t *fadeDur, const uint8_t *isNull, int sampleRate, FadePlanF32 *plans,
                            cudaStream_t stream);

cudaError_t launchKlattF32Sched(const StreamDesc *descs, uint32_t numStreams, int sampleRate, uint32_t sampleCount,
                                uint32_t holdTicks, uint32_t genTicks, int16_t *out, size_t rowStride, uint32_t *samplesWritten,
                                StreamResult *results, NoiseConfig noise, uint32_t *ring, uint32_t ringCap, void *ctlMem,
                                int16_t *scratchRow, uint32_t numBlocks, uint32_t *hostFault, void *liteMem, uint32_t holdMax,
                                uint32_t fadeTicks, uint32_t fadeMax, uint32_t roleSms, cudaStream_t stream, unsigned long long *launchCounter);
int klattF32SchedBlocksPerSm();
bool klattF32SchedUsesLite();
size_t klattF32SchedLiteBytes(uint32_t numStreams, uint32_t numBlocks);

cudaError_t launchKlattF32Block(const StreamDesc *descs, uint32_t numStreams, int sampleRate, uint32_t sampleCount, uint32_t holdTicks,
                                int16_t *out, size_t rowStride, uint32_t *samplesWritten, StreamResult *results, NoiseConfig noise,
                                void *liteMem, int16_t *scratchRow, uint32_t numBlocks, void *profMem, uint32_t *hostFault,
                                cudaStream_t stream, unsigned long long *launchCounter);
bool klattF32BlockCanTake(uint32_t numStreams, uint32_t numBlocks);
size_t klattF32BlockLiteBytes(uint32_t numStreams, uint32_t numBlocks);
cudaError_t launchKlattLiteImport(const StreamDesc *descs, uint32_t numStreams, uint32_t numDummies, void *lite, cudaStream_t stream);
cudaError_t launchKlattLiteExport(const StreamDesc *descs, uint32_t numStreams, const void *lite, uint32_t *samplesWritten, StreamResult *results,
                                  cudaStream_t stream);

cudaError_t launchKlattPullInit(PullState *state, cudaStream_t stream);
cudaError_t launchKlattPull(PullCtx ctx, const PullSeg *segSrc, int16_t *pcmOut, cudaStream_t stream);
cudaError_t launchKlattPullBatch(PullBatchItem *hItems, const PullBatchItem *dItems, uint32_t count, cudaStream_t stream);

struct LongStream {
	const double *frames;
	const uint32_t *minDur, *fadeDur;
	const uint8_t *isNull;
	const FadePlanF32 *plans;
	uint32_t nReq;
	int sampleRate;
	uint64_t seed, streamId;
	uint64_t cap;
	uint64_t outBase;
	uint64_t *start;
	int32_t *prevReal;
	double *pitchPop;
	double *pitchOld, *pitchNew, *pitchInc;
	uint64_t *vibPosStart;
};

struct LongTable {
	const LongStream *streams;
	const uint32_t *chunkBase;
	uint32_t numStreams;
	LongStream one;
};

struct Affine {
	float p00, p01, p10, p11, zy, zd;
};

cudaError_t launchKlattLongTimeline(const LongTable &T, cudaStream_t stream);
cudaError_t launchKlattLongPhase(const LongTable &T, uint32_t numChunks, uint32_t chunkTicks, uint64_t *advance, uint64_t *startPhase,
                                 PhaseChunk *chunks, double *startP, uint32_t *fail, bool serial, unsigned long long *launchCounter,
                                 cudaStream_t stream);
cudaError_t launchKlattLongSynth(const LongTable &T, uint32_t numChunks, uint32_t chunkTicks, const PhaseChunk *chunks,
                                 const double *startP, uint32_t *fail, float *ci, float *pin, float *par, float *xa, float *xb,
                                 Affine *maps, float2 *startState, void *scanScratch, int16_t *pcm, unsigned long long *launchCounter,
                                 cudaStream_t stream);
size_t klattLongScanScratchBytes(uint64_t numChunks);

}
```

Measured before the change: 3.276 million.

## Split general-render ring into tick-length bands to batch streams with similar needs

Adds a per-stream estimate of how many general-path ticks are needed before the stream can return to the cheap hold path, then routes general streams into up to six band rings keyed by that estimate (default edges 64..320 ticks). Each claimed warp renders only its band's tick count, so lanes that need few ticks no longer pad to the full general window, and all 32 lanes stay similarly busy. The push is rewritten with match_any to handle an arbitrary number of rings, and the control block grows. In exchange it adds more rings to poll, spreads streams thinner across rings so fewer full 32-lane batches form, and adds classification work after every chunk.

After: 3.267 million, median of 6. About the same (-0.3%).

```diff
diff --git a/nvspeechplayer_b200/csrc/host.cu b/nvspeechplayer_b200/csrc/host.cu
--- a/nvspeechplayer_b200/csrc/host.cu
+++ b/nvspeechplayer_b200/csrc/host.cu
@@ -78,6 +78,21 @@
 	schedGenTicks = std::max<uint32_t>(envNum<uint32_t>("NVSP_SCHED_GEN_TICKS", 384) & ~63u, 64);
 	schedHoldTicks = std::max<uint32_t>(envNum<uint32_t>("NVSP_SCHED_HOLD_TICKS", 256) & ~63u, 64);
 	schedHoldMax = std::max<uint32_t>(envNum<uint32_t>("NVSP_SCHED_HOLD_MAX", 4096) & ~63u, schedHoldTicks);
+	{
+		const char *e = getenv("NVSP_SCHED_GEN_BANDS");
+		const char *v = (e && *e) ? e : "64,128,192,256,320";
+		schedGenBands = 0;
+		if (strcmp(v, "0") != 0) {
+			schedGenBands = kSchedGenBandsOn;
+			for (uint32_t k = 0; k + 1 < kSchedRings - 2 && *v; ++k) {
+				char *end = nullptr;
+				const uint32_t edge = (uint32_t)strtoul(v, &end, 0) / 64u;
+				if (end == v) break;
+				if (edge >= 1u && edge <= 31u) schedGenBands |= 1u << (edge - 1u);
+				v = *end == ',' ? end + 1 : end;
+			}
+		}
+	}
 	schedFadeTicks = envNum<uint32_t>("NVSP_SCHED_FADE_TICKS", 0) & ~63u;
 	schedFadeMax = std::min<uint32_t>(std::max<uint32_t>(envNum<uint32_t>("NVSP_SCHED_FADE_MAX", 512) & ~63u, schedFadeTicks), 4096);
 	schedRoleSms = std::min<uint32_t>(envNum<uint32_t>("NVSP_SCHED_HOLD_SMS", 0), 255u) |
@@ -89,8 +104,8 @@
 	schedBlocks = envNum<uint32_t>("NVSP_SCHED_BLOCKS", (uint32_t)(sms * std::max(perSm, 1)));
 	blockBlocks = std::max<uint32_t>(envNum<uint32_t>("NVSP_BLOCK_BLOCKS", (uint32_t)sms), 1);
 	if (envIs("NVSP_VERBOSE"))
-		fprintf(stderr, "[nvspeechplayer_b200] scheduler: %d SMs x %d blocks, %u blocks, hold %u / general %u ticks\n", sms, perSm,
-		        schedBlocks, schedHoldTicks, schedGenTicks);
+		fprintf(stderr, "[nvspeechplayer_b200] scheduler: %d SMs x %d blocks, %u blocks, hold %u / general %u ticks, general bands 0x%08x\n",
+		        sms, perSm, schedBlocks, schedHoldTicks, schedGenTicks, schedGenBands);
 	if (!cudaOk(cudaEventCreateWithFlags(&evStart, cudaEventDisableTiming), "cudaEventCreate")) return false;
 	for (uint32_t g = 0; g < groups; ++g) {
 		if (!cudaOk(cudaStreamCreateWithFlags(&lanes[2 * g], cudaStreamNonBlocking), "cudaStreamCreate")) return false;
@@ -144,14 +159,14 @@
 		uint32_t cap = 64;
 		while (cap < 2 * n) cap <<= 1;
 		if (cudaError_t e = rc->checkFault()) return e;
-		if (!rc->ring.reserve(sizeof(uint32_t) * 3 * (size_t)cap) || !rc->ctl.reserve(2048) ||
+		if (!rc->ring.reserve(sizeof(uint32_t) * kSchedRings * (size_t)cap) || !rc->ctl.reserve(kSchedCtlBytes) ||
 		    !rc->scratchRow.reserve(sizeof(int16_t) * (size_t)std::max(std::max(std::max(rc->schedHoldTicks, rc->schedHoldMax), rc->holdTicks), rc->schedFadeMax)))
 			return cudaErrorMemoryAllocation;
 		if (klattF32SchedUsesLite() && !rc->lite.reserve(klattF32SchedLiteBytes(n, rc->schedBlocks))) return cudaErrorMemoryAllocation;
 		return launchKlattF32Sched(descs, n, sampleRate, sampleCount, rc->schedHoldTicks, rc->schedGenTicks, out, rowStride, written,
 		                           results, noise, rc->ring.as<uint32_t>(), cap, rc->ctl.p, rc->scratchRow.as<int16_t>(),
 		                           rc->schedBlocks, rc->hostFault.as<uint32_t>(), rc->lite.p, rc->schedHoldMax, rc->schedFadeTicks,
-		                           rc->schedFadeMax, rc->schedRoleSms, stream, launchCounter);
+		                           rc->schedFadeMax, rc->schedRoleSms, rc->schedGenBands, stream, launchCounter);
 	}
 	if (rc && planned && rc->init() && n >= rc->minStreams && sampleCount > rc->genTicks) {
 		const uint32_t rounds = (sampleCount + rc->genTicks - 1) / rc->genTicks;
diff --git a/nvspeechplayer_b200/csrc/host.h b/nvspeechplayer_b200/csrc/host.h
--- a/nvspeechplayer_b200/csrc/host.h
+++ b/nvspeechplayer_b200/csrc/host.h
@@ -114,6 +114,7 @@
 	uint32_t blockHoldTicks = 128, blockMinStreams = 16384, blockBlocks = 0;
 	PinnedBuf hostFault;
 	uint32_t schedHoldTicks = 256, schedGenTicks = 384, schedHoldMax = 4096, schedFadeTicks = 0, schedFadeMax = 512, schedRoleSms = 0, schedBlocks = 0;
+	uint32_t schedGenBands = 0;
 	cudaStream_t lanes[2 * kMaxGroups] = {};
 	cudaEvent_t evStart = nullptr, evFork[kMaxGroups] = {}, evJoin[kMaxGroups] = {};
 	uint32_t holdTicks = 512, genTicks = 256, minStreams = 2048, groups = 4;
diff --git a/nvspeechplayer_b200/csrc/klatt_f32_core.cuh b/nvspeechplayer_b200/csrc/klatt_f32_core.cuh
--- a/nvspeechplayer_b200/csrc/klatt_f32_core.cuh
+++ b/nvspeechplayer_b200/csrc/klatt_f32_core.cuh
@@ -541,6 +541,34 @@
 KLATT_HD bool canFadeF32T(const FM &fm, const GS &gs, uint32_t ticks) {
 	return fm.hasNew && !fm.purgePending && fm.counter >= 1 && (uint64_t)fm.counter + ticks < (uint64_t)fm.newF &&
 	       (gs.samplesGenerated & (uint64_t)(kCoarseTicks - 1)) == 0;
+}
+template <class FM, class GS>
+KLATT_HD uint32_t generalNeedT(const FM &fm, const GS &gs, const StreamDesc &desc, uint32_t sampleCount, uint32_t holdTicks,
+                               uint32_t genTicks) {
+	const uint32_t c = fm.counter, left = sampleCount - gs.callPos;
+	uint32_t need = genTicks;
+	if (!fm.purgePending) {
+		const uint32_t M = fm.hasNew ? fm.newM : fm.oldM;
+		const uint32_t ne = gs.nextEvent > c + 1u ? gs.nextEvent : c + 1u;
+		const uint32_t first = fm.hasNew ? fm.newF + 2u : gs.holdArmed ? c + 1u : ne;
+		const uint32_t T = (first - c + 63u) & ~63u;
+		if (!gs.holdArmed && first <= M && c + T + holdTicks <= M) {
+			need = T;
+		} else {
+			const uint32_t P = (M + 1u > first ? M + 1u : first) - c;
+			const uint32_t rel = fm.qHead - desc.qBase;
+			if (rel >= desc.qCount) {
+				need = P;
+			} else if (P < genTicks) {
+				const uint32_t M2 = desc.minDur[rel], F2 = desc.fadeDur[rel] > 1u ? desc.fadeDur[rel] : 1u;
+				const uint32_t T2 = (P + F2 + 2u + 63u) & ~63u;
+				if (F2 + 2u <= M2 && T2 - P + holdTicks <= M2) need = T2;
+			}
+		}
+	}
+	if (need + holdTicks > left) need = left;
+	need = (need + 63u) & ~63u;
+	return need < genTicks ? need : genTicks;
 }
 
 template <int ROLE, class Out, class Xchg, class FM, class GS>
diff --git a/nvspeechplayer_b200/csrc/klatt_f32_sched.cu b/nvspeechplayer_b200/csrc/klatt_f32_sched.cu
--- a/nvspeechplayer_b200/csrc/klatt_f32_sched.cu
+++ b/nvspeechplayer_b200/csrc/klatt_f32_sched.cu
@@ -22,20 +22,18 @@
 #endif
 
 constexpr uint32_t kRingEmpty = 0xffffffffu, kRingAbandoned = 0xfffffffeu;
-constexpr uint32_t kClassHold = 0, kClassGen = 1, kClassFade = 2, kClassExit = 3, kNumRings = 3;
+constexpr uint32_t kClassHold = 0, kClassFade = 1, kClassGen = 2, kMaxGenBands = 6, kNumRings = kClassGen + kMaxGenBands,
+                   kClassExit = kNumRings;
 
 struct SchedCtl {
-	uint32_t head0, padA[31];
-	uint32_t head1, padB[31];
-	uint32_t tail0, padC[31];
-	uint32_t tail1, padD[31];
 	uint32_t remaining, padE[31];
 	uint32_t fault, padF[31];
-	uint32_t head2, padG[31];
-	uint32_t tail2, padH[31];
-	__device__ __forceinline__ uint32_t *head(uint32_t c) { return c == 0 ? &head0 : c == 1 ? &head1 : &head2; }
-	__device__ __forceinline__ uint32_t *tail(uint32_t c) { return c == 0 ? &tail0 : c == 1 ? &tail1 : &tail2; }
+	struct Line { uint32_t v, pad[31]; } headL[kNumRings], tailL[kNumRings];
+	__device__ __forceinline__ uint32_t *head(uint32_t c) { return &headL[c].v; }
+	__device__ __forceinline__ uint32_t *tail(uint32_t c) { return &tailL[c].v; }
 };
+constexpr uint32_t kSchedProfWords = 20;
+static_assert(sizeof(SchedCtl) + 8 * kSchedProfWords <= kSchedCtlBytes, "launch.h sizes the control block");
 
 constexpr unsigned long long kWatchdogNs = 20ull * 1000 * 1000 * 1000;
 
@@ -61,6 +59,16 @@
 __device__ __forceinline__ uint32_t classifyNext(const StreamState *st, uint32_t sampleCount, uint32_t holdTicks) {
 	return classifyNextT(st->fm, st->gen.f32, sampleCount, holdTicks, 0u);
 }
+template <class FM, class GS>
+__device__ __forceinline__ uint32_t ringNextT(const FM &fm, const GS &gs, const StreamDesc &desc, uint32_t sampleCount, uint32_t holdTicks,
+                                              uint32_t genTicks, uint32_t fadeTicks, uint32_t genBands) {
+	const uint32_t cls = classifyNextT(fm, gs, sampleCount, holdTicks, fadeTicks);
+	if (cls != kClassGen || genBands == 0u) return cls;
+	const uint32_t need = generalNeedT(fm, gs, desc, sampleCount, holdTicks, genTicks);
+	const uint32_t k = need / 64u - 1u < 31u ? need / 64u - 1u : 31u;
+	const uint32_t b = __popc(genBands & ~kSchedGenBandsOn & ((1u << k) - 1u));
+	return kClassGen + (b < kMaxGenBands - 1 ? b : kMaxGenBands - 1);
+}
 constexpr uint32_t kRecPieces = sizeof(StreamStateLite) / 16, kStageStride = sizeof(StreamStateLite) + 8, kStageBytes = 32 * kStageStride;
 constexpr uint32_t kHoldPiecesOut = (uint32_t)(offsetof(StreamStateLite, f32) + offsetof(GenStateF32Lite, zre)) / 16;
 static_assert((offsetof(StreamStateLite, f32) + offsetof(GenStateF32Lite, zre)) % 16 == 0, "the hold chunk's write-back ends on a 16-byte piece");
@@ -68,23 +76,16 @@
 template <bool SEED>
 __device__ __forceinline__ void schedPush(SchedCtl *ctl, uint32_t *ring, uint32_t ringCap, uint32_t cls, uint32_t s, bool valid) {
 	const unsigned lane = threadIdx.x & 31u, below = (1u << lane) - 1u;
-	const unsigned mH = __ballot_sync(0xffffffffu, valid && cls == kClassHold);
-	const unsigned mG = __ballot_sync(0xffffffffu, valid && cls == kClassGen);
-	const unsigned mF = __ballot_sync(0xffffffffu, valid && cls == kClassFade);
 	const unsigned mX = __ballot_sync(0xffffffffu, valid && cls == kClassExit);
-	uint32_t baseH = 0, baseG = 0, baseF = 0;
-	if (lane == 0) {
-		if (mH) baseH = atomicAdd(ctl->tail(kClassHold), (uint32_t)__popc(mH));
-		if (mG) baseG = atomicAdd(ctl->tail(kClassGen), (uint32_t)__popc(mG));
-		if (mF) baseF = atomicAdd(ctl->tail(kClassFade), (uint32_t)__popc(mF));
-	}
-	baseH = __shfl_sync(0xffffffffu, baseH, 0);
-	baseG = __shfl_sync(0xffffffffu, baseG, 0);
-	baseF = __shfl_sync(0xffffffffu, baseF, 0);
+	const unsigned mine = __match_any_sync(0xffffffffu, valid ? cls : kClassExit);
+	const uint32_t leader = __ffs(mine) - 1u;
+	uint32_t base = 0;
+	if (valid && cls != kClassExit && lane == leader) base = atomicAdd(ctl->tail(cls), (uint32_t)__popc(mine));
+	base = __shfl_sync(0xffffffffu, base, leader);
 	const uint32_t mask = ringCap - 1u;
 	if (valid && cls != kClassExit) {
 		uint32_t *r = ring + cls * ringCap;
-		uint32_t idx = cls == kClassHold ? baseH + __popc(mH & below) : cls == kClassGen ? baseG + __popc(mG & below) : baseF + __popc(mF & below);
+		uint32_t idx = base + __popc(mine & below);
 		if (SEED) {
 			stVolatile(r + (idx & mask), s);
 		} else {
@@ -95,13 +96,14 @@
 		}
 	}
 	if (SEED) {
-		if (lane == 0 && (mH | mG | mF)) atomicAdd(&ctl->remaining, (uint32_t)__popc(mH | mG | mF));
+		const unsigned mIn = __ballot_sync(0xffffffffu, valid && cls != kClassExit);
+		if (lane == 0 && mIn) atomicAdd(&ctl->remaining, (uint32_t)__popc(mIn));
 	} else {
 		if (lane == 0 && mX) atomicSub(&ctl->remaining, (uint32_t)__popc(mX));
 	}
 }
 
-__device__ __forceinline__ uint32_t schedClaim(SchedCtl *ctl, uint32_t *ring, uint32_t ringCap, uint32_t &s, uint32_t primary) {
+__device__ __forceinline__ uint32_t schedClaim(SchedCtl *ctl, uint32_t *ring, uint32_t ringCap, uint32_t &s, uint32_t primary, uint32_t numRings) {
 	const unsigned lane = threadIdx.x & 31u;
 	const uint32_t mask = ringCap - 1u;
 	for (;;) {
@@ -110,10 +112,14 @@
 			uint32_t backoff = 128;
 			unsigned long long idleSince = 0;
 			for (;;) {
-				int32_t b0 = (int32_t)(ldVolatile(&ctl->tail0) - ldVolatile(&ctl->head0));
-				int32_t b1 = (int32_t)(ldVolatile(&ctl->tail1) - ldVolatile(&ctl->head1));
-				int32_t b2 = (int32_t)(ldVolatile(&ctl->tail2) - ldVolatile(&ctl->head2));
-				if (b0 > 0 || b1 > 0 || b2 > 0) {
+				int32_t b[kNumRings];
+				bool any = false;
+#pragma unroll
+				for (uint32_t c = 0; c < kNumRings; ++c) {
+					b[c] = c < numRings ? (int32_t)(ldVolatile(ctl->tail(c)) - ldVolatile(ctl->head(c))) : 0;
+					any |= b[c] > 0;
+				}
+				if (any) {
 					uint32_t pick = kClassGen;
 					int32_t best = -1;
 					bool bestFull = false;
@@ -122,12 +128,18 @@
 						const bool full = backlog >= 32;
 						if (best < 0 || (full && !bestFull) || (full == bestFull && score > best)) { pick = c; best = score; bestFull = full; }
 					};
-					consider(kClassGen, b1, 2 * b1);
-					consider(kClassFade, b2, 2 * b2);
-					consider(kClassHold, b0, b0);
+#pragma unroll
+					for (uint32_t c = kClassGen; c < kNumRings; ++c) consider(c, b[c], 2 * b[c]);
+					consider(kClassFade, b[kClassFade], 2 * b[kClassFade]);
+					consider(kClassHold, b[kClassHold], b[kClassHold]);
 					if (primary < kNumRings) {
-						const int32_t bp = primary == kClassHold ? b0 : primary == kClassGen ? b1 : b2;
-						if (bp >= 32 || (bp > 0 && !bestFull)) pick = primary;
+						uint32_t pc = primary;
+						int32_t bp = 0;
+#pragma unroll
+						for (uint32_t c = 0; c < kNumRings; ++c) {
+							if (c == primary || (primary == kClassGen && c > kClassGen && b[c] > bp)) { pc = c; bp = b[c]; }
+						}
+						if (bp >= 32 || (bp > 0 && !bestFull)) pick = pc;
 					}
 					cls = pick;
 					base = atomicAdd(ctl->head(cls), 32u);
@@ -170,7 +182,7 @@
 				else if ((spins & 15u) == 15u)
 				{
 					quit = ldVolatile(&ctl->remaining) == 0u;
-					for (uint32_t c = 0; c < kNumRings; ++c)
+					for (uint32_t c = 0; c < numRings; ++c)
 						if (c != cls && (int32_t)(ldVolatile(ctl->tail(c)) - ldVolatile(ctl->head(c))) >= 32) quit = 1u;
 				}
 			}
@@ -192,18 +204,19 @@
 
 __global__ void __launch_bounds__(256)
 klatt_sched_seed_kernel(const StreamDesc *__restrict__ descs, const StreamStateLite *__restrict__ lite, uint32_t numStreams,
-                        uint32_t sampleCount, uint32_t holdTicks, uint32_t fadeTicks, SchedCtl *ctl, uint32_t *ring, uint32_t ringCap) {
+                        uint32_t sampleCount, uint32_t holdTicks, uint32_t genTicks, uint32_t fadeTicks, uint32_t genBands, SchedCtl *ctl,
+                        uint32_t *ring, uint32_t ringCap) {
 	const uint32_t s = blockIdx.x * blockDim.x + threadIdx.x;
 	const bool valid = s < numStreams;
 	uint32_t cls = kClassExit;
 	if (valid) {
 		if (lite) {
-			cls = classifyNextT(lite[s].fm, lite[s].f32, sampleCount, holdTicks, fadeTicks);
+			cls = ringNextT(lite[s].fm, lite[s].f32, descs[s], sampleCount, holdTicks, genTicks, fadeTicks, genBands);
 		} else {
 			StreamState *st = descs[s].state;
 			st->gen.f32.callPos = 0;
 			st->gen.f32.callDrained = 0;
-			cls = classifyNext(st, sampleCount, holdTicks);
+			cls = ringNextT(st->fm, st->gen.f32, descs[s], sampleCount, holdTicks, genTicks, 0u, genBands);
 		}
 	}
 	schedPush<true>(ctl, ring, ringCap, cls, s, valid);
@@ -216,7 +229,7 @@
 klatt_f32_sched_kernel(const StreamDesc *__restrict__ descs, StreamStateLite *__restrict__ lite, uint32_t numStreams, int sampleRate,
                        uint32_t sampleCount, uint32_t holdTicks, uint32_t genTicks, int16_t *__restrict__ out, size_t rowStride,
                        int16_t *__restrict__ scratchRow, NoiseConfig noise, SchedCtl *ctl, uint32_t *ring, uint32_t ringCap,
-                       uint32_t roleSms, uint32_t holdMax, uint32_t fadeTicks, uint32_t fadeMax) {
+                       uint32_t roleSms, uint32_t holdMax, uint32_t fadeTicks, uint32_t fadeMax, uint32_t genBands) {
 	extern __shared__ uint4 schedSmem[];
 	uint4 (*xbuf)[2 * kGroupTicks * 32] = reinterpret_cast<uint4 (*)[2 * kGroupTicks * 32]>(schedSmem);
 	__shared__ uint32_t work[2][34];
@@ -231,8 +244,11 @@
 #endif
 #ifdef KLATT_SCHED_PROFILE
 	long long tClaim = 0, tHold = 0, tGen = 0, tFade = 0, tPush = 0, nHold = 0, nGen = 0, nLanes = 0;
+	long long kHold = 0, kGen = 0, kGenLoop = 0;
 	long long t0 = clock64();
 #endif
+	const uint32_t usedBands = genBands != 0u ? __popc(genBands & ~kSchedGenBandsOn) + 1u : 1u;
+	const uint32_t numRings = kClassGen + (usedBands < kMaxGenBands ? usedBands : kMaxGenBands);
 	uint32_t primary = kClassExit;
 	if (roleSms) {
 		uint32_t smid, nsm;
@@ -249,7 +265,7 @@
 	for (;;) {
 		if (cascade) {
 			uint32_t s = kRingEmpty;
-			const uint32_t cls = schedClaim(ctl, ring, ringCap, s, primary);
+			const uint32_t cls = schedClaim(ctl, ring, ringCap, s, primary, numRings);
 			if (s == kRingEmpty) s = numStreams;
 			__threadfence();
 			work[pair][lane] = s;
@@ -294,6 +310,9 @@
 				if (can > ticks) ticks = can;
 			}
 #endif
+#ifdef KLATT_SCHED_PROFILE
+			kHold += (long long)ticks * __popc(__ballot_sync(0xffffffffu, valid));
+#endif
 			if (cascade) {
 				int16_t *row = valid ? out + (size_t)s * rowStride + gs.callPos : scratchRow;
 				OutWriter ow;
@@ -327,10 +346,16 @@
 			}
 		} else {
 			const uint32_t pos = gs.callPos;
+			uint32_t loopTicks = genTicks;
+			if (genBands != 0u && cls < kNumRings - 1) {
+				uint32_t edges = genBands & ~kSchedGenBandsOn;
+				for (uint32_t b = kClassGen; b < cls; ++b) edges &= edges - 1u;
+				if (edges != 0u && 64u * (uint32_t)__ffs(edges) < genTicks) loopTicks = 64u * (uint32_t)__ffs(edges);
+			}
 			uint32_t ticks = 0;
 			if (valid) {
 				ticks = sampleCount - pos;
-				if (ticks > genTicks) ticks = genTicks;
+				if (ticks > loopTicks) ticks = loopTicks;
 				if (fadeTicks != 0u) {
 					const uint64_t end = gs.samplesGenerated + ticks, grid = end & ~(uint64_t)(kCoarseTicks - 1);
 					if (grid > gs.samplesGenerated && pos + ticks < sampleCount) ticks = (uint32_t)(grid - gs.samplesGenerated);
@@ -342,17 +367,21 @@
 				int16_t *row = out + (size_t)(valid ? s : 0) * rowStride;
 				OutWriter ow;
 				ow.init(row + pos, ((reinterpret_cast<uintptr_t>(row + pos) & 15u) == 0));
-				const uint32_t produced = renderGeneralF32T<kRoleCascade>(fm, gs, desc, sampleRate, ticks, genTicks, ow, noise, xc, &lastUserIndex, &qHead);
+				const uint32_t produced = renderGeneralF32T<kRoleCascade>(fm, gs, desc, sampleRate, ticks, loopTicks, ow, noise, xc, &lastUserIndex, &qHead);
 				ow.flush();
 				if (produced < ticks) zeroRow(row, pos + produced, sampleCount);
 			} else {
 				NullOut no;
-				renderGeneralF32T<kRoleParallel>(fm, gs, desc, sampleRate, ticks, genTicks, no, noise, xc, &lastUserIndex, &qHead);
-			}
+				renderGeneralF32T<kRoleParallel>(fm, gs, desc, sampleRate, ticks, loopTicks, no, noise, xc, &lastUserIndex, &qHead);
+			}
+#ifdef KLATT_SCHED_PROFILE
+			kGen += __reduce_add_sync(0xffffffffu, ticks);
+			kGenLoop += loopTicks;
+#endif
 		}
 #if KLATT_SCHED_LITE
 		xc.sync();
-		const uint32_t next = (cascade && valid) ? classifyNextT(fm, gs, sampleCount, holdTicks, fadeTicks) : kClassExit;
+		const uint32_t next = (cascade && valid) ? ringNextT(fm, gs, desc, sampleCount, holdTicks, genTicks, fadeTicks, genBands) : kClassExit;
 		const uint32_t piecesOut = cls == kClassHold ? kHoldPiecesOut : kRecPieces;
 #pragma unroll 1
 		for (uint32_t idx = tw; idx < 32u * piecesOut; idx += 64u) {
@@ -373,7 +402,7 @@
 #endif
 		if (cascade) {
 #if !KLATT_SCHED_LITE
-			const uint32_t next = valid ? classifyNext(desc.state, sampleCount, holdTicks) : kClassExit;
+			const uint32_t next = valid ? ringNextT(desc.state->fm, desc.state->gen.f32, desc, sampleCount, holdTicks, genTicks, 0u, genBands) : kClassExit;
 #endif
 			schedPush<false>(ctl, ring, ringCap, next, s, valid);
 		}
@@ -381,11 +410,12 @@
 	}
 #ifdef KLATT_SCHED_PROFILE
 	if (lane == 0) {
-		unsigned long long *p = reinterpret_cast<unsigned long long *>(ctl) + 128 + (cascade ? 0 : 8);
+		unsigned long long *q = reinterpret_cast<unsigned long long *>(ctl + 1), *p = q + (cascade ? 0 : 8);
 		atomicAdd(p + 0, (unsigned long long)tClaim); atomicAdd(p + 1, (unsigned long long)tHold);
 		atomicAdd(p + 2, (unsigned long long)tGen); atomicAdd(p + 3, (unsigned long long)tPush);
 		atomicAdd(p + 4, (unsigned long long)nHold); atomicAdd(p + 5, (unsigned long long)nGen);
 		atomicAdd(p + 6, (unsigned long long)nLanes); atomicAdd(p + 7, (unsigned long long)tFade);
+		if (cascade) { atomicAdd(q + 16, (unsigned long long)kHold); atomicAdd(q + 17, (unsigned long long)kGen); atomicAdd(q + 18, (unsigned long long)kGenLoop); }
 	}
 #endif
 }
@@ -402,7 +432,9 @@
                                 uint32_t holdTicks, uint32_t genTicks, int16_t *out, size_t rowStride, uint32_t *samplesWritten,
                                 StreamResult *results, NoiseConfig noise, uint32_t *ring, uint32_t ringCap, void *ctlMem,
                                 int16_t *scratchRow, uint32_t numBlocks, uint32_t *hostFault, void *liteMem, uint32_t holdMax,
-                                uint32_t fadeTicks, uint32_t fadeMax, uint32_t roleSms, cudaStream_t stream, unsigned long long *launchCounter) {
+                                uint32_t fadeTicks, uint32_t fadeMax, uint32_t roleSms, uint32_t genBands, cudaStream_t stream,
+                                unsigned long long *launchCounter) {
+	static_assert(kNumRings == kSchedRings, "launch.h sizes the ring scratch");
 	if (numStreams == 0 || sampleCount == 0) return cudaSuccess;
 	SchedCtl *ctl = static_cast<SchedCtl *>(ctlMem);
 	StreamStateLite *lite = KLATT_SCHED_LITE ? static_cast<StreamStateLite *>(liteMem) : nullptr;
@@ -415,11 +447,12 @@
 	if (!lite) fadeTicks = 0;
 	cudaError_t e = cudaMemsetAsync(ring, 0xff, sizeof(uint32_t) * kNumRings * (size_t)ringCap, stream);
 	if (e != cudaSuccess) return e;
-	if ((e = cudaMemsetAsync(ctl, 0, 2048, stream)) != cudaSuccess) return e;
+	if ((e = cudaMemsetAsync(ctl, 0, kSchedCtlBytes, stream)) != cudaSuccess) return e;
 	const uint32_t batches = (numStreams + 31) / 32;
 	const uint32_t blocksWanted = (batches + 1) / 2, grid = blocksWanted < numBlocks ? blocksWanted : numBlocks;
 	if (lite && (e = launchKlattLiteImport(descs, numStreams, 2 * grid, lite, stream)) != cudaSuccess) return e;
-	klatt_sched_seed_kernel<<<(numStreams + 255) / 256, 256, 0, stream>>>(descs, lite, numStreams, sampleCount, holdTicks, fadeTicks, ctl, ring, ringCap);
+	klatt_sched_seed_kernel<<<(numStreams + 255) / 256, 256, 0, stream>>>(descs, lite, numStreams, sampleCount, holdTicks, genTicks, fadeTicks, genBands,
+	                                                                       ctl, ring, ringCap);
 	static const bool l2Persist = getenv("NVSP_L2_PERSIST") && atoi(getenv("NVSP_L2_PERSIST")) != 0;
 	bool windowSet = false;
 	if (lite && l2Persist) {
@@ -444,7 +477,8 @@
 		}
 	}
 	klatt_f32_sched_kernel<<<grid, kPairBlock, schedSmemBytes(), stream>>>(descs, lite, numStreams, sampleRate, sampleCount, holdTicks, genTicks,
-	                                                                        out, rowStride, scratchRow, noise, ctl, ring, ringCap, roleSms, holdMax, fadeTicks, fadeMax);
+	                                                                        out, rowStride, scratchRow, noise, ctl, ring, ringCap, roleSms, holdMax, fadeTicks, fadeMax,
+	                                                                        genBands);
 	if (windowSet) {
 		cudaStreamAttrValue attr;
 		memset(&attr, 0, sizeof attr);
@@ -461,13 +495,15 @@
 	}
 #ifdef KLATT_SCHED_PROFILE
 	{
-		unsigned long long h[16];
+		unsigned long long h[kSchedProfWords];
 		cudaStreamSynchronize(stream);
-		cudaMemcpy(h, reinterpret_cast<unsigned long long *>(ctl) + 128, sizeof(h), cudaMemcpyDeviceToHost);
+		cudaMemcpy(h, ctl + 1, sizeof(h), cudaMemcpyDeviceToHost);
 		for (int k = 0; k < 2; ++k)
 			fprintf(stderr, "[sched profile] %s warps: claim %.1f  hold %.1f  gen %.1f  fade %.1f  push %.1f Mcycles; batches hold %llu gen+fade %llu; lanes/batch %.2f\n",
 			        k ? "parallel" : "cascade ", h[8 * k] / 1e6, h[8 * k + 1] / 1e6, h[8 * k + 2] / 1e6, h[8 * k + 7] / 1e6, h[8 * k + 3] / 1e6, h[8 * k + 4], h[8 * k + 5],
 			        (double)h[8 * k + 6] / (double)(h[8 * k + 4] + h[8 * k + 5]));
+		fprintf(stderr, "[sched profile] stream-ticks: hold %.4g  general %.4g (hold share %.1f %%); general loop trips %.4g, mean %.1f ticks\n",
+		        (double)h[16], (double)h[17], 100.0 * (double)h[16] / (double)(h[16] + h[17]), (double)h[18], (double)h[18] / (double)h[5]);
 	}
 #endif
 	return cudaGetLastError();
diff --git a/nvspeechplayer_b200/csrc/launch.h b/nvspeechplayer_b200/csrc/launch.h
--- a/nvspeechplayer_b200/csrc/launch.h
+++ b/nvspeechplayer_b200/csrc/launch.h
@@ -35,7 +35,11 @@
                                 uint32_t holdTicks, uint32_t genTicks, int16_t *out, size_t rowStride, uint32_t *samplesWritten,
                                 StreamResult *results, NoiseConfig noise, uint32_t *ring, uint32_t ringCap, void *ctlMem,
                                 int16_t *scratchRow, uint32_t numBlocks, uint32_t *hostFault, void *liteMem, uint32_t holdMax,
-                                uint32_t fadeTicks, uint32_t fadeMax, uint32_t roleSms, cudaStream_t stream, unsigned long long *launchCounter);
+                                uint32_t fadeTicks, uint32_t fadeMax, uint32_t roleSms, uint32_t genBands, cudaStream_t stream,
+                                unsigned long long *launchCounter);
+constexpr uint32_t kSchedRings = 8;
+constexpr size_t kSchedCtlBytes = 4096;
+constexpr uint32_t kSchedGenBandsOn = 0x80000000u;
 int klattF32SchedBlocksPerSm();
 bool klattF32SchedUsesLite();
 size_t klattF32SchedLiteBytes(uint32_t numStreams, uint32_t numBlocks);
```
